# ZhengyiLuo/SMPLSim

Measured on AMD Instinct MI355X. Metric: env-steps/sec (whole node), 4096-env SMPL rollout at 1/2/4/8 MI355X, higher is better.
Workload: dtype f32

## Files before the change

include/smplsim_hip.h:

```cpp
#ifndef SMPLSIM_HIP_H
#define SMPLSIM_HIP_H
#include <stddef.h>
#include <stdint.h>

#ifdef __cplusplus
extern "C" {
#endif

typedef enum {
  SS_OK = 0,
  SS_ERR_INVALID = -1,
  SS_ERR_HIP = -2,
  SS_ERR_NOMEM = -3,
  SS_ERR_LDS = -4
} ss_status;

enum { SS_GEOM_BOX = 0, SS_GEOM_CAPSULE = 1,
       SS_GEOM_SPHERE = 2 };
enum { SS_TASK_BASE = 0, SS_TASK_SPEED = 1, SS_TASK_GETUP = 2, SS_TASK_REACH = 3 };
enum { SS_INIT_DEFAULT = 0, SS_INIT_FALL = 1,
       SS_INIT_EXTERNAL = 2 };
enum { SS_CTRL_UHC_PD = 0, SS_CTRL_PD = 1, SS_CTRL_TORQUE = 2, SS_CTRL_SIMPLE_PID = 3, SS_CTRL_DEFAULT = 4 };

typedef struct {
  int32_t nbody;
  const int32_t *body_parent;
  const double *body_pos;
  const double *body_mass;
  const double *body_ipos;
  const double *body_iquat;
  const double *body_inertia;
  const int32_t *geom_type;
  const double *geom_size;
  const double *geom_pos;
  const double *geom_quat;
  const double *dof_armature;
  const double *jnt_range;
  const uint8_t *jnt_limited;
  const double *body_invweight0;
  const double *dof_invweight0;
  const double *qpos0;
  int32_t nu;
  const int32_t *actuator_dof;
  const double *kp, *kd, *torque_lim, *act_scale, *act_offset;
  const uint8_t *legal_contact;
  double timestep, gravity, solref[2], solimp[5], margin, friction, impratio;
  const int32_t *geom_contype;
  const int32_t *geom_conaffinity;
  int32_t nexclude;
  const int32_t *exclude;
  double meaninertia;
} ss_model_desc;

typedef struct {
  int32_t task, state_init, self_obs_v, control_mode;
  int32_t episode_length, control_freq_inv, root_height_obs;
  float power_scale;
  float tar_speed_min, tar_speed_max; int32_t speed_change_min, speed_change_max;
  float tar_height_min, tar_height_max; int32_t height_change_min, height_change_max, recovery_steps;
  int32_t newton_iters;
  float tar_dist_max; int32_t reach_body;
  int32_t self_collision;
  float solver_tolerance;
} ss_env_cfg;
#ifndef SS_MAX_SELF_CONTACTS_N
#define SS_MAX_SELF_CONTACTS_N 64
#endif
enum { SS_MAX_SELF_CONTACTS = SS_MAX_SELF_CONTACTS_N };

typedef struct {
  int32_t num_envs;
  float *qpos;
  float *qvel;
  float *qpos_prev;
  float *qvel_prev;
  float *qacc_warm;
  float *body_vel;
  int32_t *touch;
  int32_t *cur_t;
  float *task;
  int32_t *nwarn;
  int32_t *solver_iters;
  float *pid_integral;
  float *pid_last_error;
  int32_t *pid_started;
  const int32_t *shape_id;
  int32_t *self_contacts;
} ss_state;

typedef struct ss_model ss_model;
typedef struct ss_batch ss_batch;

int ss_model_create(const ss_model_desc *desc, int device_id, ss_model **out);
int ss_model_create_shapes(const ss_model_desc *descs, int32_t num_shapes, int device_id, ss_model **out);

typedef struct {
  int32_t control_mode;
  int32_t clip_actions;
  double pdp_scale, pdd_scale;
  double timestep;
  int32_t num_contact_bodies;
  const char *const *contact_bodies;
} ss_mjcf_options;
int ss_model_create_from_mjcf(const char *xml, size_t len, const ss_mjcf_options *opts, int device_id, ss_model **out);
void ss_model_destroy(ss_model *m);
int ss_model_dims(const ss_model *m, int32_t *nq, int32_t *nv, int32_t *nu, int32_t *nbody);
int ss_model_elimination_tree(const ss_model *m, int32_t *root, int32_t *levels, int32_t *widest, int32_t *widths, int32_t *most_children);
int ss_obs_size(const ss_model *m, const ss_env_cfg *cfg);

int ss_batch_create(const ss_model *m, const ss_env_cfg *cfg, const ss_state *state, ss_batch **out);
void ss_batch_destroy(ss_batch *b);

int ss_reset(ss_batch *b, const uint8_t *mask, const float *fall_actions, const float *task_rand,
             float *obs, void *stream);

int ss_step(ss_batch *b, const float *actions, const float *task_rand, float *obs, float *reward,
            uint8_t *terminated, uint8_t *truncated, void *stream);

int ss_set_order(ss_batch *b, const int32_t *order);
int ss_schedule_longest_first(ss_batch *b, void *stream);

int ss_step_autoreset(ss_batch *b, const float *actions, const float *task_rand, const float *reset_task_rand, float *obs,
                      float *obs_next, float *reward, uint8_t *terminated, uint8_t *truncated, void *stream);
int ss_set_fall_actions(ss_batch *b, const float *fall_actions);

int ss_substep(ss_batch *b, const float *actions, int n_substeps, void *stream);

int ss_kinematics(ss_batch *b, float *xpos, float *xmat, void *stream);

int ss_set_body_outputs(ss_batch *b, float *xpos, float *xmat);

int ss_set_power_output(ss_batch *b, float *power);

int ss_debug_forward(ss_batch *b, const float *torques, float *M, float *bias, float *qacc, void *stream);
int ss_debug_self_contacts(ss_batch *b, float *records);
int ss_debug_self_truncation(ss_batch *b, int32_t *counts);
int ss_gae(const float *rewards, const float *not_done, const float *not_dead, const float *values, const float *bootstrap,
           int32_t T, int32_t N, float gamma, float tau, float *advantages, float *returns, void *stream);

int ss_debug_prof(ss_batch *b, unsigned long long *out, int n);

int ss_launch_info(const ss_batch *b, int32_t *envs_per_wg, int32_t *lds_bytes, int32_t *kernel_regs);

int ss_set_launch_geometry(ss_batch *b, int32_t envs_per_wg, int32_t max_workgroups);

enum { SS_FIELD_QPOS = 0,
       SS_FIELD_QVEL = 1,
       SS_FIELD_XPOS = 2,
       SS_FIELD_XMAT = 3,
       SS_FIELD_BODY_VEL = 4,
       SS_FIELD_TOUCH = 5,
       SS_FIELD_QACC_WARM = 6,
       SS_FIELD_CUR_T = 7 };
int ss_get_state(ss_batch *b, int32_t field, void *buf, void *stream);
int ss_set_state(ss_batch *b, int32_t field, const void *buf, void *stream);


const char *ss_last_error(void);
const char *ss_model_last_error(const ss_model *m);
const char *ss_batch_last_error(const ss_batch *b);

#ifdef __cplusplus
}
#endif
#endif
```

smplsim_amd/_cabi.py:

```python
import ctypes as C

import numpy as np

TASK_BASE, TASK_SPEED, TASK_GETUP, TASK_REACH = 0, 1, 2, 3
INIT_DEFAULT, INIT_FALL, INIT_EXTERNAL = 0, 1, 2
CTRL_UHC_PD, CTRL_PD, CTRL_TORQUE, CTRL_SIMPLE_PID, CTRL_DEFAULT = 0, 1, 2, 3, 4
TASKS = {"HumanoidEnv": TASK_BASE, "HumanoidSpeed": TASK_SPEED, "HumanoidGetup": TASK_GETUP, "HumanoidReach": TASK_REACH}
CONTROL_MODES = {"uhc_pd": CTRL_UHC_PD, "pd": CTRL_PD, "torque": CTRL_TORQUE, "simple_pid": CTRL_SIMPLE_PID,
                 "default": CTRL_DEFAULT}
STATE_INITS = {"Default": INIT_DEFAULT, "Fall": INIT_FALL, "External": INIT_EXTERNAL}
SS_MAX_SELF_CONTACTS = 64


class ModelDesc(C.Structure):
    _fields_ = [
        ("nbody", C.c_int32), ("body_parent", C.c_void_p), ("body_pos", C.c_void_p), ("body_mass", C.c_void_p),
        ("body_ipos", C.c_void_p), ("body_iquat", C.c_void_p), ("body_inertia", C.c_void_p),
        ("geom_type", C.c_void_p), ("geom_size", C.c_void_p), ("geom_pos", C.c_void_p), ("geom_quat", C.c_void_p),
        ("dof_armature", C.c_void_p), ("jnt_range", C.c_void_p), ("jnt_limited", C.c_void_p),
        ("body_invweight0", C.c_void_p), ("dof_invweight0", C.c_void_p), ("qpos0", C.c_void_p),
        ("nu", C.c_int32), ("actuator_dof", C.c_void_p), ("kp", C.c_void_p), ("kd", C.c_void_p),
        ("torque_lim", C.c_void_p), ("act_scale", C.c_void_p), ("act_offset", C.c_void_p),
        ("legal_contact", C.c_void_p),
        ("timestep", C.c_double), ("gravity", C.c_double), ("solref", C.c_double * 2), ("solimp", C.c_double * 5),
        ("margin", C.c_double), ("friction", C.c_double), ("impratio", C.c_double),
        ("geom_contype", C.c_void_p), ("geom_conaffinity", C.c_void_p), ("nexclude", C.c_int32), ("exclude", C.c_void_p),
        ("meaninertia", C.c_double),
    ]


class EnvCfg(C.Structure):
    _fields_ = [
        ("task", C.c_int32), ("state_init", C.c_int32), ("self_obs_v", C.c_int32), ("control_mode", C.c_int32),
        ("episode_length", C.c_int32), ("control_freq_inv", C.c_int32), ("root_height_obs", C.c_int32),
        ("power_scale", C.c_float),
        ("tar_speed_min", C.c_float), ("tar_speed_max", C.c_float), ("speed_change_min", C.c_int32),
        ("speed_change_max", C.c_int32),
        ("tar_height_min", C.c_float), ("tar_height_max", C.c_float), ("height_change_min", C.c_int32),
        ("height_change_max", C.c_int32), ("recovery_steps", C.c_int32), ("newton_iters", C.c_int32),
        ("tar_dist_max", C.c_float), ("reach_body", C.c_int32), ("self_collision", C.c_int32),
        ("solver_tolerance", C.c_float),
    ]


class State(C.Structure):
    _fields_ = [
        ("num_envs", C.c_int32), ("qpos", C.c_void_p), ("qvel", C.c_void_p), ("qpos_prev", C.c_void_p),
        ("qvel_prev", C.c_void_p), ("qacc_warm", C.c_void_p), ("body_vel", C.c_void_p), ("touch", C.c_void_p),
        ("cur_t", C.c_void_p), ("task", C.c_void_p), ("nwarn", C.c_void_p), ("solver_iters", C.c_void_p),
        ("pid_integral", C.c_void_p), ("pid_last_error", C.c_void_p), ("pid_started", C.c_void_p), ("shape_id", C.c_void_p),
        ("self_contacts", C.c_void_p),
    ]


class Skeleton(C.Structure):
    _fields_ = [("nbody", C.c_int32), ("parent", C.c_void_p), ("smpl_2_mujoco", C.c_void_p)]


MOTION_DATA_ARRAYS = ("length_starts", "motion_num_frames", "motion_dt", "motion_lengths", "frame_motion", "pose_aa", "trans",
                      "offsets", "gts", "grs", "lrs", "gvs", "gavs", "dof_pos", "dvs", "qpos", "qvel")


class MotionData(C.Structure):
    _fields_ = [("num_motions", C.c_int32), ("num_frames", C.c_int32), ("nbody", C.c_int32)] + \
               [(n, C.c_void_p) for n in MOTION_DATA_ARRAYS]


MOTION_STATE_FIELDS = ("root_pos", "root_rot", "dof_pos", "root_vel", "root_ang_vel", "dof_vel", "rg_pos", "rb_rot", "body_vel",
                       "body_ang_vel", "qpos", "qvel")


class MotionState(C.Structure):
    _fields_ = [(n, C.c_void_p) for n in MOTION_STATE_FIELDS]


class ImitationCfg(C.Structure):
    _fields_ = [(n, C.c_float) for n in ("k_pos", "k_rot", "k_vel", "k_ang_vel", "w_pos", "w_rot", "w_vel", "w_ang_vel",
                                         "termination_distance", "obs_dt")]


class ImitationIO(C.Structure):
    _fields_ = [("data", C.POINTER(MotionData)), ("cfg", ImitationCfg), ("motion_ids", C.c_void_p), ("start_times", C.c_void_p),
                ("offset", C.c_void_p), ("sampling_cdf", C.c_void_p), ("truncate_time", C.c_float), ("random_start", C.c_int32),
                ("obs_final", C.c_void_p), ("obs_next", C.c_void_p), ("obs_stride", C.c_int32), ("reward", C.c_void_p),
                ("reward_parts", C.c_void_p), ("terminated", C.c_void_p), ("truncated", C.c_void_p)]


class MjcfOptions(C.Structure):
    _fields_ = [("control_mode", C.c_int32), ("clip_actions", C.c_int32), ("pdp_scale", C.c_double), ("pdd_scale", C.c_double),
                ("timestep", C.c_double), ("num_contact_bodies", C.c_int32), ("contact_bodies", C.POINTER(C.c_char_p))]


def bind(lib):
    vp = C.c_void_p
    lib.ss_model_create_from_mjcf.argtypes = [C.c_char_p, C.c_size_t, C.POINTER(MjcfOptions), C.c_int, C.POINTER(vp)]
    lib.ss_set_fall_actions.argtypes = [vp, vp]
    lib.ss_get_state.argtypes = [vp, C.c_int32, vp, vp]
    lib.ss_set_state.argtypes = [vp, C.c_int32, vp, vp]
    lib.ss_imitation_bind.argtypes = [vp, C.POINTER(ImitationIO)]
    lib.ss_imitation_step_fused.argtypes = [vp, vp, vp, vp]
    lib.ss_model_last_error.argtypes = [vp]; lib.ss_model_last_error.restype = C.c_char_p
    lib.ss_batch_last_error.argtypes = [vp]; lib.ss_batch_last_error.restype = C.c_char_p
    lib.ss_model_create.argtypes = [C.POINTER(ModelDesc), C.c_int, C.POINTER(vp)]
    lib.ss_model_create_shapes.argtypes = [C.POINTER(ModelDesc), C.c_int32, C.c_int, C.POINTER(vp)]
    lib.ss_model_destroy.argtypes = [vp]; lib.ss_model_destroy.restype = None
    lib.ss_model_dims.argtypes = [vp] + [C.POINTER(C.c_int32)] * 4
    lib.ss_obs_size.argtypes = [vp, C.POINTER(EnvCfg)]
    lib.ss_batch_create.argtypes = [vp, C.POINTER(EnvCfg), C.POINTER(State), C.POINTER(vp)]
    lib.ss_batch_destroy.argtypes = [vp]; lib.ss_batch_destroy.restype = None
    lib.ss_reset.argtypes = [vp, vp, vp, vp, vp, vp]
    lib.ss_step.argtypes = [vp] * 8
    lib.ss_substep.argtypes = [vp, vp, C.c_int, vp]
    lib.ss_kinematics.argtypes = [vp, vp, vp, vp]
    lib.ss_debug_forward.argtypes = [vp, vp, vp, vp, vp, vp]
    lib.ss_debug_self_contacts.argtypes = [vp, vp]
    lib.ss_debug_self_truncation.argtypes = [vp, vp]
    lib.ss_model_elimination_tree.argtypes = [vp, vp, vp, vp, vp, vp]
    lib.ss_step_autoreset.argtypes = [vp] * 10
    lib.ss_schedule_longest_first.argtypes = [vp, vp]
    lib.ss_gae.argtypes = [vp, vp, vp, vp, vp, C.c_int32, C.c_int32, C.c_float, C.c_float, vp, vp, vp]
    lib.ss_debug_prof.argtypes = [vp, vp, C.c_int]
    lib.ss_set_order.argtypes = [vp, vp]
    lib.ss_set_body_outputs.argtypes = [vp, vp, vp]
    lib.ss_set_power_output.argtypes = [vp, vp]
    lib.ss_set_launch_geometry.argtypes = [vp, C.c_int32, C.c_int32]
    lib.ss_launch_info.argtypes = [vp] + [C.POINTER(C.c_int32)] * 3
    lib.ss_last_error.argtypes = []; lib.ss_last_error.restype = C.c_char_p
    lib.ss_motion_cook.argtypes = [C.POINTER(Skeleton), C.POINTER(MotionData), C.c_int32, vp]
    lib.ss_motion_state_at.argtypes = [C.POINTER(MotionData), vp, vp, vp, vp, C.c_int32, C.c_int32, C.POINTER(MotionState), vp]
    lib.ss_motion_resample.argtypes = [C.POINTER(MotionData), vp, vp, vp, C.c_float, C.c_int32, vp, vp, vp]
    lib.ss_imitation_step.argtypes = [C.POINTER(MotionData), C.POINTER(ImitationCfg)] + [vp] * 5 + [C.c_int32] + [vp] * 4 + \
                                     [C.c_int32] + [vp] * 5
    return lib


FIELDS = {"qpos": 0, "qvel": 1, "xpos": 2, "xmat": 3, "body_vel": 4, "touch": 5, "qacc_warm": 6, "cur_t": 7}
ACTIVATIONS = {"none": 0, "silu": 1, "tanh": 2, "relu": 3}
MLP_EXPORTS = ["ss_linear_bf16", "ss_linear_bf16_train", "ss_linear_bf16_dx", "ss_wgrad_bf16", "ss_obs_to_bf16", "ss_gaussian_sample",
               "ss_debug_last_gemm", "ss_linear_bf16_dx_det", "ss_linear_bf16_dx_det_workspace", "ss_wgrad_bf16_det", "ss_wgrad_bf16_det_workspace"]


def bind_mlp(lib):
    vp = C.c_void_p
    lib.ss_linear_bf16.argtypes = [vp, vp, vp, vp, C.c_int32, C.c_int32, C.c_int32, C.c_int32, C.c_int32, C.c_int32, vp]
    lib.ss_linear_bf16_train.argtypes = [vp, vp, vp, vp, vp, vp, vp, C.c_int32, C.c_int32, C.c_int32, C.c_int32, C.c_int32, C.c_int32, C.c_int32, vp]
    lib.ss_linear_bf16_dx.argtypes = [vp, vp, vp, vp, vp, C.c_int32, C.c_int32, C.c_int32, C.c_int32, vp]
    lib.ss_wgrad_bf16.argtypes = [vp, vp, vp, C.c_int32, C.c_int32, C.c_int32, C.c_int32, C.c_int32, C.c_int32, vp]
    lib.ss_linear_bf16_dx_det.argtypes = [vp, vp, vp, vp, vp, C.c_int32, C.c_int32, C.c_int32, C.c_int32, vp, C.c_int64, vp]
    lib.ss_linear_bf16_dx_det_workspace.argtypes = [C.c_int32, C.c_int32, C.c_int32]; lib.ss_linear_bf16_dx_det_workspace.restype = C.c_int64
    lib.ss_wgrad_bf16_det.argtypes = [vp, vp, vp, C.c_int32, C.c_int32, C.c_int32, C.c_int32, C.c_int32, C.c_int32, vp, C.c_int64, vp]
    lib.ss_wgrad_bf16_det_workspace.argtypes = [C.c_int32, C.c_int32, C.c_int32]; lib.ss_wgrad_bf16_det_workspace.restype = C.c_int64
    lib.ss_obs_to_bf16.argtypes = [vp, C.c_int32, C.c_int32, C.c_int32, vp, vp, vp, C.c_float, C.c_float, C.c_float, vp, C.c_int32, vp]
    lib.ss_gaussian_sample.argtypes = [vp, vp, vp, C.c_int32, C.c_int32, vp, C.c_int32, vp, C.c_int32, C.c_float, C.c_float, vp, vp]
    lib.ss_debug_last_gemm.argtypes = [C.c_char_p, C.c_int32]
    return lib


EXPORTS = ["ss_model_create", "ss_model_create_shapes", "ss_model_destroy", "ss_model_dims", "ss_model_elimination_tree", "ss_obs_size", "ss_batch_create",
           "ss_batch_destroy", "ss_reset", "ss_step", "ss_step_autoreset", "ss_substep", "ss_kinematics", "ss_debug_forward", "ss_debug_self_contacts", "ss_debug_self_truncation",
           "ss_gae", "ss_debug_prof", "ss_set_order", "ss_set_body_outputs", "ss_set_power_output", "ss_set_launch_geometry", "ss_schedule_longest_first", "ss_launch_info", "ss_last_error",
           "ss_model_create_from_mjcf", "ss_model_last_error", "ss_batch_last_error", "ss_imitation_bind", "ss_imitation_step_fused", "ss_get_state", "ss_set_state", "ss_set_fall_actions",
           "ss_motion_cook", "ss_motion_state_at", "ss_motion_resample", "ss_imitation_step"]


def make_model_desc(mc, kp, kd, torque_lim, act_scale, act_offset, legal_bodies=(), timestep=1.0 / 450):
    keep = []

    def arr(x, dt):
        a = np.ascontiguousarray(x, dtype=dt)
        keep.append(a)
        return a.ctypes.data_as(C.c_void_p)

    d = ModelDesc()
    d.nbody = mc.nbody
    d.body_parent = arr(mc.body_parent, np.int32)
    for name in ("body_pos", "body_mass", "body_ipos", "body_iquat", "body_inertia", "geom_size", "geom_pos",
                 "geom_quat", "dof_armature", "jnt_range", "body_invweight0", "dof_invweight0", "qpos0"):
        setattr(d, name, arr(getattr(mc, name), np.float64))
    d.geom_type = arr(mc.geom_type, np.int32)
    d.jnt_limited = arr(mc.jnt_limited, np.uint8)
    d.nu = mc.nu
    d.actuator_dof = arr(mc.actuator_dof, np.int32)
    d.kp, d.kd, d.torque_lim = arr(kp, np.float64), arr(kd, np.float64), arr(torque_lim, np.float64)
    d.act_scale, d.act_offset = arr(act_scale, np.float64), arr(act_offset, np.float64)
    d.legal_contact = arr([int(n in legal_bodies) for n in mc.body_names], np.uint8)
    d.timestep, d.gravity = timestep, mc.gravity
    d.solref = (C.c_double * 2)(*mc.solref)
    d.solimp = (C.c_double * 5)(*mc.solimp)
    d.margin, d.friction, d.impratio = mc.geom_margin, mc.friction, mc.impratio
    d.geom_contype = arr(mc.geom_contype, np.int32)
    d.geom_conaffinity = arr(mc.geom_conaffinity, np.int32)
    ex = [(mc.body_names.index(a), mc.body_names.index(b)) for a, b in mc.excludes]
    d.nexclude = len(ex)
    d.exclude = arr(np.array(ex, dtype=np.int32).reshape(-1, 2), np.int32) if ex else None
    d.meaninertia = mc.meaninertia
    return d, keep


def make_env_cfg(task=TASK_BASE, state_init=INIT_DEFAULT, self_obs_v=1, control_mode=CTRL_UHC_PD,
                 episode_length=300, control_freq_inv=15, root_height_obs=True, power_scale=1.0,
                 tar_speed=(0.0, 5.0), speed_change=(100, 200), tar_height=(0.5, 1.2), height_change=(100, 200),
                 recovery_steps=60, newton_iters=0, tar_dist_max=1.0, reach_body=0, self_collision=False, solver_tolerance=0.0):
    return EnvCfg(task, state_init, self_obs_v, control_mode, episode_length, control_freq_inv, int(root_height_obs),
                  power_scale, tar_speed[0], tar_speed[1], speed_change[0], speed_change[1], tar_height[0],
                  tar_height[1], height_change[0], height_change[1], recovery_steps, newton_iters, tar_dist_max, reach_body,
                  int(bool(self_collision)), solver_tolerance)
```

smplsim_amd/batch.py:

```python
import ctypes as C
import os
import warnings

import numpy as np
import torch

from . import _cabi
from ._lib import lib
from .gains import build_pd_tables
from .mjcf import compile_mjcf
from .mjcf_writer import default_xml_str

DEFAULT_CONTACT_BODIES = ("R_Ankle", "L_Ankle", "R_Toe", "L_Toe")


def _check(rc):
    if rc != 0:
        raise RuntimeError(f"libsmplsim_hip error {rc}: {lib().ss_last_error().decode()}")


def _ptr(t):
    return None if t is None else C.c_void_p(t.data_ptr())


def _shard_device(index):
    if not torch.cuda.is_available():
        raise RuntimeError("SMPLSimVecEnv needs a ROCm GPU (MI355X); there is no CPU fallback")
    return torch.device("cuda", int(index))


def _launch_stream(device):
    return C.c_void_p(torch.cuda.current_stream(device).cuda_stream)


_WARNED = False


def _warn_floor_only():
    global _WARNED
    if not _WARNED:
        _WARNED = True
        warnings.warn("SMPLSimVecEnv(self_collision=False): floor contacts and joint limits only — bodies of the humanoid pass through "
                      "each other, unlike mj_step on the reference MJCF (contype/conaffinity, smpl_humanoid.xml:5,24). Pass "
                      "self_collision=True for the reference's contact set (about 3x the step time under violent actions).", stacklevel=3)


class ShardModel:

    def __init__(self, xml=None, humanoid="smpl_humanoid", device=0, contact_bodies=DEFAULT_CONTACT_BODIES,
                 control_mode="uhc_pd", clip_actions=True, pdp_scale=1.0, pdd_scale=1.0, sim_timestep_inv=450, tables=None, xmls=None, mcs=None, compiler="python", lazy=False):
        if mcs is not None:
            self.mcs, self.xmls = list(mcs), []
            self.xml = None
        else:
            self.xmls = list(xmls) if xmls is not None else [xml if xml is not None else default_xml_str(humanoid)]
            self.xml = self.xmls[0]
            self.mcs = [compile_mjcf(x) for x in self.xmls]
        self.mc, self.num_shapes = self.mcs[0], len(self.mcs)
        rng = {n: self.mc.jnt_range[6 + i] for i, n in enumerate(self.mc.joint_names)}
        self.tables = tables if tables is not None else build_pd_tables(
            self.mc.actuator_names, lambda n: rng[n], clip_actions=clip_actions, control_mode=control_mode,
            pdp_scale=pdp_scale, pdd_scale=pdd_scale)
        self.device = int(device)
        if compiler == "native":
            if self.num_shapes != 1 or self.xml is None or tables is not None:
                raise ValueError("compiler='native' takes one MJCF text and the reference's gain table")
        elif compiler != "python":
            raise ValueError(f"unknown compiler {compiler!r}")
        self._args = dict(compiler=compiler, contact_bodies=tuple(contact_bodies), control_mode=control_mode, clip_actions=clip_actions,
                          pdp_scale=pdp_scale, pdd_scale=pdd_scale, sim_timestep_inv=sim_timestep_inv)
        self._handle, self._pid = None, None
        if not lazy:
            self.handle

    @property
    def handle(self):
        if self._handle is None or self._pid != os.getpid():
            a = self._args
            h = C.c_void_p()
            if a["compiler"] == "native":
                names = (C.c_char_p * len(a["contact_bodies"]))(*[n.encode() for n in a["contact_bodies"]])
                opt = _cabi.MjcfOptions(_cabi.CONTROL_MODES[a["control_mode"]], int(bool(a["clip_actions"])), a["pdp_scale"], a["pdd_scale"],
                                        1.0 / a["sim_timestep_inv"], len(a["contact_bodies"]), names)
                txt = self.xml.encode()
                _check(lib().ss_model_create_from_mjcf(txt, len(txt), C.byref(opt), self.device, C.byref(h)))
            else:
                descs, self._keep = (_cabi.ModelDesc * self.num_shapes)(), []
                for i, mc in enumerate(self.mcs):
                    descs[i], keep = _cabi.make_model_desc(mc, *self.tables, legal_bodies=a["contact_bodies"], timestep=1.0 / a["sim_timestep_inv"])
                    self._keep.append(keep)
                _check(lib().ss_model_create_shapes(descs, self.num_shapes, self.device, C.byref(h)))
            self._handle, self._pid = h, os.getpid()
        return self._handle

    def __del__(self):
        h = getattr(self, "_handle", None)
        if h and getattr(self, "_pid", None) == os.getpid():
            try:
                lib().ss_model_destroy(h)
            except Exception:
                pass


class SMPLSimVecEnv:

    def __init__(self, num_envs, model=None, device=0, task="HumanoidEnv", state_init="Default", self_obs_v=1,
                 control_mode="uhc_pd", episode_length=300, control_freq_inv=15, root_height_obs=True,
                 power_scale=1.0, tar_speed=(0.0, 5.0), speed_change=(100, 200), tar_height=(0.5, 1.2),
                 height_change=(100, 200), recovery_steps=60, tar_dist_max=1.0, reach_body="R_Hand", newton_iters=0, fused_autoreset=True,
                 autoreset=True, seed=0, lpt_order=True, shape_id=None, self_collision=False, solver_tolerance=0.0,
                 **model_kw):
        self.device = _shard_device(device if model is None else model.device)
        self.model = model if model is not None else ShardModel(device=device, control_mode=control_mode, **model_kw)
        mc = self.model.mc
        self.num_envs = int(num_envs)
        self.nq, self.nv, self.nu, self.nbody = mc.nq, mc.nv, mc.nu, mc.nbody
        self.task_id = _cabi.TASKS[task] if isinstance(task, str) else int(task)
        if self.task_id == _cabi.TASK_REACH and isinstance(reach_body, str) and reach_body not in mc.body_names:
            raise ValueError(f"reach_body {reach_body!r} is not a body of this model")
        self.state_init = _cabi.STATE_INITS[state_init] if isinstance(state_init, str) else int(state_init)
        if self.state_init == _cabi.INIT_EXTERNAL and autoreset:
            raise ValueError("StateInit External keeps the state the caller wrote: pass autoreset=False and reset finished envs "
                             "yourself (write qpos / qvel, then reset(mask)), as SMPLSimImitationVecEnv does")
        self.cfg = _cabi.make_env_cfg(
            task=self.task_id, state_init=self.state_init, self_obs_v=self_obs_v,
            control_mode=_cabi.CONTROL_MODES[control_mode], episode_length=episode_length,
            control_freq_inv=control_freq_inv, root_height_obs=root_height_obs, power_scale=power_scale,
            tar_speed=tar_speed, speed_change=speed_change, tar_height=tar_height, height_change=height_change,
            recovery_steps=recovery_steps, newton_iters=newton_iters, tar_dist_max=tar_dist_max,
            reach_body=self._body_index(mc, reach_body), self_collision=self_collision, solver_tolerance=solver_tolerance)
        self.self_collision = bool(self_collision)
        if not self.self_collision:
            _warn_floor_only()
        N, dev = self.num_envs, self.device
        f32 = dict(dtype=torch.float32, device=dev)
        i32 = dict(dtype=torch.int32, device=dev)
        self.qpos = torch.zeros(N, self.nq, **f32); self.qvel = torch.zeros(N, self.nv, **f32)
        self.qpos_prev = torch.zeros(N, self.nq, **f32); self.qvel_prev = torch.zeros(N, self.nv, **f32)
        self.qacc_warm = torch.zeros(N, self.nv, **f32); self.body_vel = torch.zeros(N, self.nbody, 6, **f32)
        self.touch = torch.zeros(N, 2, **i32); self.cur_t = torch.zeros(N, **i32)
        self.task_state = torch.zeros(N, 4, **f32); self.nwarn = torch.zeros(N, **i32)
        self.solver_iters = torch.zeros(N, **i32)
        self.pid_integral = torch.zeros(N, self.nu, **f32); self.pid_last_error = torch.zeros(N, self.nu, **f32)
        self.pid_started = torch.zeros(N, **i32)
        self.self_contacts = torch.zeros(N, **i32)
        self.qpos[:, 3] = 1; self.qpos_prev[:, 3] = 1
        self.shape_id = None
        if self.model.num_shapes > 1:
            sid = torch.arange(N, device=dev) % self.model.num_shapes if shape_id is None else torch.as_tensor(shape_id, device=dev)
            if sid.shape != (N,) or int(sid.min()) < 0 or int(sid.max()) >= self.model.num_shapes:
                raise ValueError("shape_id must hold one shape index in [0, num_shapes) per env")
            self.shape_id = sid.to(torch.int32).contiguous()
        elif shape_id is not None:
            raise ValueError("shape_id given but the model has a single shape (build it with ShardModel(xmls=[...]))")
        st = _cabi.State(N, *[_ptr(t) for t in (self.qpos, self.qvel, self.qpos_prev, self.qvel_prev, self.qacc_warm,
                                               self.body_vel, self.touch, self.cur_t, self.task_state, self.nwarn,
                                               self.solver_iters, self.pid_integral, self.pid_last_error,
                                               self.pid_started, self.shape_id, self.self_contacts)])
        self.handle = C.c_void_p()
        _check(lib().ss_batch_create(self.model.handle, C.byref(self.cfg), C.byref(st), C.byref(self.handle)))
        self.obs_size = lib().ss_obs_size(self.model.handle, C.byref(self.cfg))
        self.obs_buf = torch.zeros(N, self.obs_size, **f32)
        self.rew_buf = torch.zeros(N, **f32)
        self.terminated = torch.zeros(N, dtype=torch.uint8, device=dev)
        self.truncated = torch.zeros(N, dtype=torch.uint8, device=dev)
        self.reset_buf = torch.zeros(N, dtype=torch.uint8, device=dev)
        self.obs_final = torch.zeros(N, self.obs_size, **f32)
        self._fused_autoreset = self.state_init in (_cabi.INIT_DEFAULT, _cabi.INIT_FALL) and fused_autoreset
        self._fall_buf = None
        if self._fused_autoreset and self.state_init == _cabi.INIT_FALL:
            self._fall_buf = torch.zeros(N, 3, self.nu, **f32)
            _check(lib().ss_set_fall_actions(self.handle, _ptr(self._fall_buf)))
        self.autoreset = autoreset
        self.gen = torch.Generator(device=dev)
        self.gen.manual_seed(int(seed))
        self.action_size = self.nu
        self.actuator_names = list(mc.actuator_names)
        self._keep = self._keep2 = None
        self.lpt_order = bool(lpt_order) and N > 64
        self.order = torch.arange(N, dtype=torch.int32, device=dev)

    @staticmethod
    def _body_index(mc, body):
        if not isinstance(body, str):
            return int(body)
        if body in mc.body_names:
            return mc.body_names.index(body)
        return 0

    def _task_rand(self):
        if self.task_id == _cabi.TASK_BASE:
            return None
        return torch.rand(self.num_envs, 4, generator=self.gen, device=self.device)

    def _fall_actions(self):
        if self.state_init != _cabi.INIT_FALL:
            return None
        return torch.rand(self.num_envs, 3, self.nu, generator=self.gen, device=self.device)

    def _stream(self):
        return _launch_stream(self.device)

    def reset(self, mask=None, fall_actions=None, task_rand=None):
        fa = fall_actions if fall_actions is not None else self._fall_actions()
        tr = task_rand if task_rand is not None else self._task_rand()
        m = None if mask is None else mask.to(torch.uint8).contiguous()
        self._keep = (fa, tr, m)
        _check(lib().ss_reset(self.handle, _ptr(m), _ptr(fa), _ptr(tr), _ptr(self.obs_buf), self._stream()))
        return self.obs_buf, {"critic_state": self.obs_buf}

    def step(self, actions, task_rand=None, _events=None, task_rand2=None, _fall_drawn=False):
        actions = actions.to(torch.float32).contiguous()
        assert actions.shape == (self.num_envs, self.nu) and actions.device == self.device
        tr = task_rand if task_rand is not None else self._task_rand()
        self._keep = (actions, tr)
        if self.lpt_order:
            _check(lib().ss_schedule_longest_first(self.handle, self._stream()))
        if _events:
            _events[0].record()
        info = {}
        if self.autoreset and self._fused_autoreset:
            tr2 = task_rand2 if task_rand2 is not None else self._task_rand()
            self._keep2 = (tr2,)
            if self._fall_buf is not None and not _fall_drawn:
                self._fall_buf.uniform_(0.0, 1.0, generator=self.gen)
            _check(lib().ss_step_autoreset(self.handle, _ptr(actions), _ptr(tr), _ptr(tr2), _ptr(self.obs_final), _ptr(self.obs_buf),
                                           _ptr(self.rew_buf), _ptr(self.terminated), _ptr(self.truncated), self._stream()))
            if _events:
                _events[1].record()
            if self.lpt_order:
                _check(lib().ss_set_order(self.handle, None))
            info["final_observation"] = self.obs_final
            info["critic_state"] = self.obs_buf
            return self.obs_buf, self.rew_buf, self.terminated.bool(), self.truncated.bool(), info
        _check(lib().ss_step(self.handle, _ptr(actions), _ptr(tr), _ptr(self.obs_buf), _ptr(self.rew_buf),
                             _ptr(self.terminated), _ptr(self.truncated), self._stream()))
        if _events:
            _events[1].record()
        if self.lpt_order:
            _check(lib().ss_set_order(self.handle, None))
        if self.autoreset:
            torch.bitwise_or(self.terminated, self.truncated, out=self.reset_buf)
            info["final_observation"] = self.obs_buf.clone()
            fa, tr2 = self._fall_actions(), self._task_rand()
            self._keep2 = (fa, tr2)
            _check(lib().ss_reset(self.handle, _ptr(self.reset_buf), _ptr(fa), _ptr(tr2), _ptr(self.obs_buf),
                                  self._stream()))
        info["critic_state"] = self.obs_buf
        return self.obs_buf, self.rew_buf, self.terminated.bool(), self.truncated.bool(), info

    def substep(self, actions, n):
        actions = actions.to(torch.float32).contiguous()
        self._keep = (actions,)
        _check(lib().ss_substep(self.handle, _ptr(actions), int(n), self._stream()))

    def kinematics(self):
        xpos = torch.zeros(self.num_envs, self.nbody, 3, device=self.device)
        xmat = torch.zeros(self.num_envs, self.nbody, 9, device=self.device)
        _check(lib().ss_kinematics(self.handle, _ptr(xpos), _ptr(xmat), self._stream()))
        return xpos, xmat

    def enable_power_usage(self):
        if getattr(self, "power_usage", None) is None:
            self.power_usage = torch.zeros(self.num_envs, int(self.cfg.control_freq_inv), self.nv - 6, device=self.device)
            _check(lib().ss_set_power_output(self.handle, _ptr(self.power_usage)))
        return self.power_usage

    def debug_forward(self, torques=None):
        M = torch.zeros(self.num_envs, self.nv, self.nv, device=self.device)
        bias = torch.zeros(self.num_envs, self.nv, device=self.device)
        qacc = torch.zeros(self.num_envs, self.nv, device=self.device)
        tq = None if torques is None else torques.to(torch.float32).contiguous()
        _check(lib().ss_debug_forward(self.handle, _ptr(tq), _ptr(M), _ptr(bias), _ptr(qacc), self._stream()))
        return M, bias, qacc

    def debug_self_contacts(self):
        if getattr(self, "self_records", None) is None:
            self.self_records = torch.zeros(self.num_envs, _cabi.SS_MAX_SELF_CONTACTS, 24, device=self.device)
            _check(lib().ss_debug_self_contacts(self.handle, _ptr(self.self_records)))
        return self.self_records

    def set_state(self, qpos, qvel, qpos_prev=None, qvel_prev=None, warm=None):
        def as_t(x):
            if torch.is_tensor(x):
                return x.to(self.device, torch.float32)
            return torch.as_tensor(np.asarray(x), dtype=torch.float32, device=self.device)
        self.qpos.copy_(as_t(qpos)); self.qvel.copy_(as_t(qvel))
        self.qpos_prev.copy_(as_t(qpos if qpos_prev is None else qpos_prev))
        self.qvel_prev.copy_(as_t(qvel if qvel_prev is None else qvel_prev))
        if warm is not None:
            self.qacc_warm.copy_(as_t(warm))

    def launch_info(self):
        a, b, c = C.c_int32(), C.c_int32(), C.c_int32()
        _check(lib().ss_launch_info(self.handle, C.byref(a), C.byref(b), C.byref(c)))
        return {"envs_per_workgroup": a.value, "lds_bytes": b.value, "vgprs": c.value}

    def close(self):
        h = getattr(self, "handle", None)
        if h:
            if self.device.type == "cuda":
                torch.cuda.synchronize(self.device)
            lib().ss_batch_destroy(h)
            self.handle = None

    def __del__(self):
        try:
            self.close()
        except Exception:
            pass
```

smplsim_amd/csrc/smplsim_hip.hip:

```cpp
#include <hip/hip_runtime.h>

#include "ss_env_kernel.h"

namespace {


__global__ void ss_gae_kernel(const float *rew, const float *nd, const float *ndead, const float *val, const float *boot,
                              int T, int N, float gamma, float tau, float *adv, float *ret) {
  const int n = blockIdx.x * blockDim.x + threadIdx.x;
  if (n >= N) return;
  float next_v = boot ? boot[n] : 0.f, next_a = 0.f;
  for (int t = T - 1; t >= 0; --t) {
    const size_t i = (size_t)t * N + n;
    const float v = val[i];
    const float delta = rew[i] + gamma * next_v * ndead[i] - v;
    const float a = delta + gamma * tau * next_a * nd[i];
    adv[i] = a; ret[i] = v + a;
    next_v = v; next_a = a;
  }
}

__global__ void __launch_bounds__(256) ss_key_kernel(const float *qvel, const float *qacc, const int32_t *touch, const int32_t *iters, int nv, int n,
                                                     int32_t *key) {
  const int env = blockIdx.x * 4 + (threadIdx.x >> 6), lane = threadIdx.x & 63;
  if (env >= n) return;
  float vm = 0.f, am = 0.f;
  for (int i = lane; i < nv; i += 64) {
    const float v = fabsf(qvel[(size_t)env * nv + i]), a = fabsf(qacc[(size_t)env * nv + i]);
    vm = fmaxf(vm, v == v ? v : 1e6f); am = fmaxf(am, a == a ? a : 1e12f);
  }
  for (int m = 32; m >= 1; m >>= 1) { vm = fmaxf(vm, __shfl_xor(vm, m, 64)); am = fmaxf(am, __shfl_xor(am, m, 64)); }
  if (lane == 0) {
    const int tc = __popc((unsigned)touch[2 * env]) + __popc((unsigned)touch[2 * env + 1]);
    const float k = (float)iters[env] + 6.f * (float)tc + 8.f * log1pf(fminf(am, 1e12f)) + 8.f * log1pf(fminf(vm, 1e6f));
    key[env] = (int32_t)fminf(fmaxf(k, 0.f), 1023.f);
  }
}

__global__ void __launch_bounds__(1024) ss_order_kernel(const int32_t *keys, int32_t *order, int n) {
  __shared__ int hist[1024], offs[1024];
  for (int i = threadIdx.x; i < 1024; i += blockDim.x) hist[i] = 0;
  __syncthreads();
  for (int i = threadIdx.x; i < n; i += blockDim.x) { int key = keys[i]; key = key < 0 ? 0 : (key > 1023 ? 1023 : key); atomicAdd(&hist[1023 - key], 1); }
  __syncthreads();
  if (threadIdx.x < 32) {
    int acc = 0;
    for (int i = 0; i < 32; i++) { const int h_ = hist[threadIdx.x * 32 + i]; offs[threadIdx.x * 32 + i] = acc; acc += h_; }
    int base = 0;
    for (int l = 0; l < 32; l++) { const int t = __shfl(acc, l, 64); if (l < (int)threadIdx.x) base += t; }
    for (int i = 0; i < 32; i++) offs[threadIdx.x * 32 + i] += base;
  }
  __syncthreads();
  for (int i = threadIdx.x; i < n; i += blockDim.x) { int key = keys[i]; key = key < 0 ? 0 : (key > 1023 ? 1023 : key); order[atomicAdd(&offs[1023 - key], 1)] = i; }
}


typedef ss::kern_t kern_t;
kern_t pick_kernel(int variant, int flavour, const ss::Hdr &h, const ss::HdrC &hc) {
#ifndef SS_NO_FIXED_LAYOUT
  if (variant == 0 && flavour == 0 && HdrSmpl::matches(h, hc)) return ss_env_kernel<2, 2, 1, 1, SS_MAX_THREADS, false, false, HdrSmpl>;
#ifndef SS_ONLY_HEADLINE
  if (variant == 0 && flavour == 1 && HdrSmpl::matches(h, hc)) return ss_env_kernel<2, 2, 1, 1, SS_MAX_THREADS, true, false, HdrSmpl>;
  if (variant == 0 && flavour == 2 && HdrSmpl::matches(h, hc)) return ss_env_kernel<2, 2, 1, 1, SS_MAX_THREADS, true, true, HdrSmpl>;
#endif
#endif
  if (variant == 0 && flavour == 0) return ss_env_kernel<2, 2, 1, 1, SS_MAX_THREADS, false, false>;
#ifndef SS_ONLY_HEADLINE
  if (flavour == 3 || flavour == 5 || flavour == 7) return ss::pick_kernel_selfcol(variant, flavour == 5, flavour == 7, h, hc);
  if (flavour == 4 || flavour == 6) return ss::pick_kernel_imitation(variant, flavour == 6, h, hc);
  if (variant == 0) {
    if (flavour == 1) return ss_env_kernel<2, 2, 1, 1, SS_MAX_THREADS, true, false>;
    return ss_env_kernel<2, 2, 1, 1, SS_MAX_THREADS, true, true>;
  }
  if (variant == 1) return ss::pick_kernel_x(flavour, h, hc);
#endif
  return nullptr;
}

struct HipBackend {
  static void *alloc(size_t n) { void *p = nullptr; return hipMalloc(&p, n) == hipSuccess ? p : nullptr; }
  static void free_(void *p) { if (p) (void)hipFree(p); }
  static bool upload(void *dst, const void *src, size_t n) { return hipMemcpy(dst, src, n, hipMemcpyHostToDevice) == hipSuccess; }
  static bool set_device(int d) { return hipSetDevice(d) == hipSuccess; }
  static bool download(void *dst, const void *src, size_t n) { return hipMemcpy(dst, src, n, hipMemcpyDeviceToHost) == hipSuccess; }
  static bool copy_d2d(void *dst, const void *src, size_t n, void *stream) { return hipMemcpyAsync(dst, src, n, hipMemcpyDeviceToDevice, (hipStream_t)stream) == hipSuccess; }
  static int lds_capacity() { return 160 * 1024; }
  static int num_cus() { int d = 0, n = 256; if (hipGetDevice(&d) == hipSuccess) { hipDeviceProp_t p; if (hipGetDeviceProperties(&p, d) == hipSuccess) n = p.multiProcessorCount; } return n; }
  static int max_waves(int variant, int selfcol) { return (variant == 0 ? (selfcol ? SS_MAX_THREADS_SC : SS_MAX_THREADS) : SS_MAX_THREADS_X) / 64; }
  static const char *order_by_key(const ss_state &st, int nv, int32_t *key, int32_t *order, void *stream) {
    const int n = st.num_envs;
    hipLaunchKernelGGL(ss_key_kernel, dim3((n + 3) / 4), dim3(256), 0, (hipStream_t)stream, st.qvel, st.qacc_warm, st.touch, st.solver_iters, nv, n, key);
    hipLaunchKernelGGL(ss_order_kernel, dim3(1), dim3(1024), 0, (hipStream_t)stream, key, order, n);
    hipError_t e = hipGetLastError();
    return e == hipSuccess ? nullptr : hipGetErrorString(e);
  }
  static const char *gae(const float *rew, const float *nd, const float *ndead, const float *val, const float *boot, int T, int N,
                         float gamma, float tau, float *adv, float *ret, void *stream) {
    hipLaunchKernelGGL(ss_gae_kernel, dim3((N + 255) / 256), dim3(256), 0, (hipStream_t)stream, rew, nd, ndead, val, boot, T, N, gamma, tau, adv, ret);
    hipError_t e = hipGetLastError();
    return e == hipSuccess ? nullptr : hipGetErrorString(e);
  }
  static int &regs_ref() { static thread_local int r = 0; return r; }
  static int kernel_regs() { return regs_ref(); }
  static const char *launch(const ss::KArgs &k, int nenv, int envs_per_wg, size_t lds_bytes, void *stream, int fixed_epw, int max_wgs) {
    const bool bodyout = (k.out0 || k.power) && (k.mode == ss::MODE_STEP || k.mode == ss::MODE_RESET);
    const int flavour = k.im ? (k.cfg.self_collision ? 7 : (k.st.shape_id ? 6 : 4)) : (k.cfg.self_collision ? (k.st.shape_id ? 5 : 3) : (k.st.shape_id ? 2 : (bodyout ? 1 : 0)));
    kern_t kern = pick_kernel(ss::kernel_variant(k.h), flavour, k.h, k.hc);
    if (!kern) return "no kernel variant for this model size";
    static thread_local kern_t configured[32] = {};
    static thread_local size_t configured_lds[32] = {};
    static thread_local int regs_by_slot[32] = {};
    const int slot = 16 * ss::kernel_variant(k.h) + flavour;
    if (configured[slot] != kern || configured_lds[slot] < lds_bytes) {
      hipError_t e = hipFuncSetAttribute(reinterpret_cast<const void *>(kern), hipFuncAttributeMaxDynamicSharedMemorySize, (int)lds_bytes);
      if (e != hipSuccess) return hipGetErrorString(e);
      hipFuncAttributes fa;
      if (hipFuncGetAttributes(&fa, reinterpret_cast<const void *>(kern)) == hipSuccess) regs_by_slot[slot] = fa.numRegs;
      configured[slot] = kern; configured_lds[slot] = lds_bytes;
    }
    regs_ref() = regs_by_slot[slot];
    static thread_local int cus = num_cus();
    const int per_cu = (nenv + cus - 1) / cus;
    if (fixed_epw > 0) {
      envs_per_wg = fixed_epw;
      lds_bytes = ss::launch_lds_bytes(k, envs_per_wg);
    } else if (per_cu < envs_per_wg) {
      envs_per_wg = per_cu < 1 ? 1 : per_cu;
      lds_bytes = ss::launch_lds_bytes(k, envs_per_wg);
    }
    int wgs = (nenv + envs_per_wg - 1) / envs_per_wg;
    const int resident = cus * (int)(lds_capacity() / lds_bytes > 0 ? lds_capacity() / lds_bytes : 1);
    if (wgs > resident) wgs = resident;
    if (max_wgs > 0 && wgs > max_wgs) wgs = max_wgs;
    dim3 grid(wgs), block(64 * envs_per_wg);
    hipLaunchKernelGGL(kern, grid, block, lds_bytes, (hipStream_t)stream, k);
    hipError_t e = hipGetLastError();
    return e == hipSuccess ? nullptr : hipGetErrorString(e);
  }
};

}

SS_DEFINE_C_API(HipBackend)
```

smplsim_amd/csrc/ss_api.h:

```cpp
#pragma once
#include <cstdlib>
#include <new>
#include <string>

#include "ss_imfused.h"
#include "ss_mjcf.h"
#include "ss_tables.h"

namespace ss {
inline std::string &last_error() { static thread_local std::string e; return e; }
inline std::string *&error_slot() { static thread_local std::string *p = nullptr; return p; }
struct HandleScope {
  explicit HandleScope(std::string *slot) { error_slot() = slot; }
  ~HandleScope() { error_slot() = nullptr; }
};
}

struct ss_model {
  ss::HostModel hm;
  int device = 0;
  uint32_t *d_shared = nullptr;
  ss::real *d_bodyc = nullptr, *d_candc = nullptr;
  int32_t *d_candb = nullptr;
  int32_t *d_pairs = nullptr;
  ss::real *d_geomc = nullptr;
  int num_shapes = 1;
  mutable std::string err;
};
struct ss_batch {
  const ss_model *m = nullptr;
  ss_env_cfg cfg{};
  ss_state st{};
  int envs_per_wg = 1;
  size_t lds_bytes = 0;
  int obs_size = 0;
  int32_t *d_counter = nullptr;
  unsigned long long *d_prof = nullptr;
  const int32_t *order = nullptr;
  int32_t *d_sched = nullptr;
  float *body_xpos = nullptr, *body_xmat = nullptr;
  static ss::real *R(float *p) { return reinterpret_cast<ss::real *>(p); }
  static const ss::real *R(const float *p) { return reinterpret_cast<const ss::real *>(p); }
  float *dbg_self = nullptr;
  int32_t *self_trunc = nullptr;
  float *power = nullptr;
  int fixed_envs_per_wg = 0, max_wgs = 0;
  mutable std::string err;
  mutable int kernel_regs = 0;
  mutable int parity = 0;
  float *d_kin = nullptr;
  const float *fall_actions = nullptr;
  void *d_im = nullptr;
  ss_imitation_io im_io{};
};

inline bool same_pair_ids(const std::vector<int32_t> &a, const std::vector<int32_t> &b) {
  if (a.size() != b.size()) return false;
  for (size_t i = 0; i < a.size(); i += 2) if (a[i] != b[i]) return false;
  return true;
}

template <class BE>
struct ss_api {
  static int fail(int code, const std::string &msg) {
    ss::last_error() = msg;
    if (ss::error_slot()) *ss::error_slot() = msg;
    return code;
  }

  static int model_create(const ss_model_desc *d, int device, ss_model **out) {
    if (!d || !out) return fail(SS_ERR_INVALID, "null argument");
    ss_model *m = new (std::nothrow) ss_model();
    if (!m) return fail(SS_ERR_NOMEM, "out of host memory");
    if (!ss::build_host_model(*d, m->hm)) { std::string e = m->hm.error; delete m; return fail(SS_ERR_INVALID, e); }
    m->device = device;
    if (!BE::set_device(device)) { delete m; return fail(SS_ERR_HIP, "cannot select device"); }
    auto up = [&](const void *src, size_t bytes) -> void * {
      void *p = BE::alloc(bytes ? bytes : 4);
      if (p && bytes && !BE::upload(p, src, bytes)) { BE::free_(p); p = nullptr; }
      return p;
    };
    m->d_shared = (uint32_t *)up(m->hm.shared.data(), m->hm.shared.size() * 4);
    m->d_bodyc = (ss::real *)up(m->hm.bodyc.data(), m->hm.bodyc.size() * sizeof(ss::real));
    m->d_candc = (ss::real *)up(m->hm.candc.data(), m->hm.candc.size() * sizeof(ss::real));
    m->d_candb = (int32_t *)up(m->hm.candb.data(), m->hm.candb.size() * 4);
    {
      std::vector<int32_t> pt(m->hm.pairs);
      m->hm.sc.o_sctab = (int)pt.size();
      pt.insert(pt.end(), m->hm.sctab.begin(), m->hm.sctab.end());
      m->d_pairs = (int32_t *)up(pt.data(), pt.size() * 4);
    }
    m->d_geomc = (ss::real *)up(m->hm.geomc.data(), m->hm.geomc.size() * sizeof(ss::real));
    if (!m->d_shared || !m->d_bodyc || !m->d_candc || !m->d_candb || !m->d_pairs || !m->d_geomc) { model_destroy(m); return fail(SS_ERR_HIP, "device table upload failed"); }
    *out = m;
    return SS_OK;
  }
  static int model_create_shapes(const ss_model_desc *d, int num_shapes, int device, ss_model **out) {
    if (!d || !out || num_shapes < 1) return fail(SS_ERR_INVALID, "null argument or num_shapes < 1");
    if (num_shapes == 1) return model_create(d, device, out);
    ss_model *m = new (std::nothrow) ss_model();
    if (!m) return fail(SS_ERR_NOMEM, "out of host memory");
    std::vector<ss::real> bodyc, candc, geomc;
    std::vector<int32_t> pairs;
    for (int s = 0; s < num_shapes; s++) {
      ss::HostModel hm;
      if (!ss::build_host_model(d[s], hm)) { std::string e = "shape " + std::to_string(s) + ": " + hm.error; delete m; return fail(SS_ERR_INVALID, e); }
      const ss::Hdr &h = hm.h;
      std::vector<ss::real> iw(h.nv);
      ss::real *sf = ss::shared_reals(hm);
      for (int i = 0; i < h.nv; i++) { iw[i] = sf[h.o_dofc + i * ss::kDofC + 4]; sf[h.o_dofc + i * ss::kDofC + 4] = 0; }
      for (int i = 0; i < 3 * h.nb; i++) sf[h.o_boff + i] = 0;
      if (s == 0) m->hm = hm;
      else {
        const ss::Hdr &g = m->hm.h;
        const bool same = h.nb == g.nb && h.nv == g.nv && h.nu == g.nu && h.ncand == g.ncand && h.nbox == g.nbox && h.nslot == g.nslot &&
                          h.shared_words == g.shared_words && h.env_floats == g.env_floats && hm.shared == m->hm.shared &&
                          hm.candb == m->hm.candb && same_pair_ids(hm.pairs, m->hm.pairs) && hm.illegal_mask == m->hm.illegal_mask && h.dt == g.dt && h.grav == g.grav &&
                          h.margin == g.margin && h.mu == g.mu && h.K == g.K && h.B == g.B;
        if (!same) { delete m; return fail(SS_ERR_INVALID, "shape " + std::to_string(s) + " differs from shape 0 in more than its geometry"); }
      }
      bodyc.insert(bodyc.end(), hm.bodyc.begin(), hm.bodyc.end());
      iw.resize((h.nv + 3) & ~3, ss::real(0));
      bodyc.insert(bodyc.end(), iw.begin(), iw.end());
      candc.insert(candc.end(), hm.candc.begin(), hm.candc.end());
      geomc.insert(geomc.end(), hm.geomc.begin(), hm.geomc.end());
      pairs.insert(pairs.end(), hm.pairs.begin(), hm.pairs.end());
    }
    if (12 * m->hm.h_sc.nb > m->hm.h_sc.l_Wst - m->hm.h_sc.l_IA) { delete m; return fail(SS_ERR_LDS, "no room for the per-env body offsets"); }
    m->device = device; m->num_shapes = num_shapes;
    if (!BE::set_device(device)) { delete m; return fail(SS_ERR_HIP, "cannot select device"); }
    auto up = [&](const void *src, size_t bytes) -> void * {
      void *p = BE::alloc(bytes ? bytes : 4);
      if (p && bytes && !BE::upload(p, src, bytes)) { BE::free_(p); p = nullptr; }
      return p;
    };
    m->d_shared = (uint32_t *)up(m->hm.shared.data(), m->hm.shared.size() * 4);
    m->d_bodyc = (ss::real *)up(bodyc.data(), bodyc.size() * sizeof(ss::real));
    m->d_candc = (ss::real *)up(candc.data(), candc.size() * sizeof(ss::real));
    m->d_candb = (int32_t *)up(m->hm.candb.data(), m->hm.candb.size() * 4);
    m->hm.sc.o_sctab = (int)pairs.size();
    pairs.insert(pairs.end(), m->hm.sctab.begin(), m->hm.sctab.end());
    m->d_pairs = (int32_t *)up(pairs.data(), pairs.size() * 4);
    m->d_geomc = (ss::real *)up(geomc.data(), geomc.size() * sizeof(ss::real));
    if (!m->d_shared || !m->d_bodyc || !m->d_candc || !m->d_candb || !m->d_pairs || !m->d_geomc) { model_destroy(m); return fail(SS_ERR_HIP, "device table upload failed"); }
    *out = m;
    return SS_OK;
  }
  static void model_destroy(ss_model *m) {
    if (!m) return;
    BE::free_(m->d_shared); BE::free_(m->d_bodyc); BE::free_(m->d_candc); BE::free_(m->d_candb); BE::free_(m->d_pairs); BE::free_(m->d_geomc);
    delete m;
  }
  static int batch_create(const ss_model *m, const ss_env_cfg *cfg, const ss_state *st, ss_batch **out) {
    if (!m || !cfg || !st || !out) return fail(SS_ERR_INVALID, "null argument");
    if (st->num_envs < 1) return fail(SS_ERR_INVALID, "num_envs must be positive");
    if (!st->qpos || !st->qvel || !st->qpos_prev || !st->qvel_prev || !st->qacc_warm || !st->body_vel || !st->touch ||
        !st->cur_t || !st->task || !st->nwarn || !st->solver_iters)
      return fail(SS_ERR_INVALID, "every ss_state buffer must be provided");
    if (cfg->control_mode < SS_CTRL_UHC_PD || cfg->control_mode > SS_CTRL_DEFAULT) return fail(SS_ERR_INVALID, "unknown control_mode");
    if (cfg->control_mode == SS_CTRL_SIMPLE_PID && (!st->pid_integral || !st->pid_last_error || !st->pid_started))
      return fail(SS_ERR_INVALID, "control_mode simple_pid needs the pid_* state buffers");
    if (cfg->self_obs_v != 1 && cfg->self_obs_v != 2) return fail(SS_ERR_INVALID, "self_obs_v must be 1 or 2");
    if (cfg->control_freq_inv < 1) return fail(SS_ERR_INVALID, "control_freq_inv must be >= 1");
    if (m->num_shapes > 1 && !st->shape_id) return fail(SS_ERR_INVALID, "a model with several shapes needs ss_state.shape_id");
    if (m->num_shapes == 1 && st->shape_id) return fail(SS_ERR_INVALID, "ss_state.shape_id given for a single-shape model");
    if (cfg->self_collision && !m->d_pairs) return fail(SS_ERR_INVALID, "model has no pair table");
    if (cfg->self_collision && !m->hm.self_collision_unavailable.empty()) return fail(SS_ERR_INVALID, m->hm.self_collision_unavailable.c_str());
    if (cfg->task == SS_TASK_REACH && (cfg->reach_body < 0 || cfg->reach_body >= m->hm.h.nb)) return fail(SS_ERR_INVALID, "reach_body out of range");
    const ss::Hdr &h = m->hm.h;
    if (ss::kernel_variant(h) < 0) return fail(SS_ERR_INVALID, "model too large for the compiled kernel variants");
    ss_batch *b = new (std::nothrow) ss_batch();
    if (!b) return fail(SS_ERR_NOMEM, "out of host memory");
    b->m = m; b->cfg = *cfg; b->st = *st;
    if (b->cfg.newton_iters <= 0) b->cfg.newton_iters = 100;
    b->cfg.solver_tolerance = (float)((cfg->solver_tolerance > 0.f ? (double)cfg->solver_tolerance : 1e-8) * m->hm.meaninertia * (h.nv > 1 ? h.nv : 1));
    b->obs_size = ss::obs_size(h, *cfg);
    size_t shared_b = (size_t)((h.shared_words + 3) & ~3) * 4;
    const size_t env_b = (size_t)(cfg->self_collision ? m->hm.sc.env_floats : h.env_floats) * sizeof(ss::real);
    int cap = BE::lds_capacity();
    const size_t pool_b = cfg->self_collision ? (size_t)ss::ss_pool_floats(m->hm.sc) * sizeof(ss::real) : 0;
    int e = (int)((cap - (long)shared_b - (long)pool_b) / (long)env_b);
    if (e < 1) { delete b; return fail(SS_ERR_LDS, "model does not fit in LDS"); }
    { const int mw = BE::max_waves(ss::kernel_variant(h), cfg->self_collision); if (e > mw) e = mw; }
    { const char *cap = getenv("SS_ENVS_PER_WG"); if (cap && atoi(cap) > 0 && atoi(cap) < e) e = atoi(cap); }
    b->envs_per_wg = e;
    b->lds_bytes = shared_b + (size_t)e * env_b + pool_b;
#ifdef SS_PROFILE
    b->d_prof = (unsigned long long *)BE::alloc(64 * sizeof(unsigned long long));
    if (b->d_prof) { unsigned long long z[64] = {0}; BE::upload(b->d_prof, z, sizeof z); }
#endif
    if (!BE::set_device(m->device)) { delete b; return fail(SS_ERR_HIP, "cannot select device"); }
    b->d_counter = (int32_t *)BE::alloc(2 * sizeof(int32_t));
    const int32_t zeros[2] = {0, 0};
    if (!b->d_counter || !BE::upload(b->d_counter, zeros, sizeof zeros)) { BE::free_(b->d_counter); delete b; return fail(SS_ERR_NOMEM, "device allocation failed"); }
    *out = b;
    return SS_OK;
  }
  static ss::KArgs base_args(const ss_batch *b, int mode) {
    ss::KArgs k{};
    const ss_model *m = b->m;
    k.h = b->cfg.self_collision ? m->hm.h_sc : m->hm.h; k.cfg = b->cfg; k.st = b->st;
    k.shared_g = m->d_shared; k.bodyc = m->d_bodyc; k.candc = m->d_candc; k.candb = m->d_candb;
    k.illegal_mask = m->hm.illegal_mask;
    k.hc = m->hm.hc;
    k.sc = m->hm.sc; k.pairs = m->d_pairs; k.geomc = m->d_geomc; k.dbg_self = ss_batch::R(b->dbg_self);
    k.mode = mode; k.nsub = b->cfg.control_freq_inv; k.obs_size = b->obs_size;
    k.work_counter = b->d_counter + b->parity; k.work_counter_next = b->d_counter + (b->parity ^ 1);
    k.obs_stride = b->obs_size;
    k.prof = b->d_prof;
    k.order = b->order;
    if (mode == ss::MODE_STEP || mode == ss::MODE_RESET) { k.out0 = ss_batch::R(b->body_xpos); k.out1 = ss_batch::R(b->body_xmat); }
    if (mode == ss::MODE_STEP) { k.power = ss_batch::R(b->power); k.self_trunc = b->self_trunc; }
    return k;
  }
  static int run(const ss_batch *b, const ss::KArgs &k, void *stream) {
    if (!BE::set_device(b->m->device)) return fail(SS_ERR_HIP, "cannot select device");
    const char *err = BE::launch(k, b->st.num_envs, b->envs_per_wg, b->lds_bytes, stream, b->fixed_envs_per_wg, b->max_wgs);
    if (err) return fail(SS_ERR_HIP, err);
    b->kernel_regs = BE::kernel_regs();
    b->parity ^= 1;
    return SS_OK;
  }
  static int reset(ss_batch *b, const uint8_t *mask, const float *fall_actions, const float *task_rand, float *obs, void *stream) {
    if (!b || !obs) return fail(SS_ERR_INVALID, "null argument");
    if (b->cfg.state_init == SS_INIT_FALL && !fall_actions) return fail(SS_ERR_INVALID, "StateInit.Fall needs fall_actions");
    ss::KArgs k = base_args(b, ss::MODE_RESET);
    k.mask = mask; k.fall_actions = ss_batch::R(fall_actions); k.task_rand = ss_batch::R(task_rand); k.obs = ss_batch::R(obs);
    return run(b, k, stream);
  }
  static int step(ss_batch *b, const float *actions, const float *task_rand, float *obs, float *reward, uint8_t *term,
                  uint8_t *trunc, void *stream) {
    if (!b || !actions || !obs || !reward || !term || !trunc) return fail(SS_ERR_INVALID, "null argument");
    ss::KArgs k = base_args(b, ss::MODE_STEP);
    k.actions = ss_batch::R(actions); k.task_rand = ss_batch::R(task_rand); k.obs = ss_batch::R(obs); k.reward = ss_batch::R(reward);
    k.terminated = term; k.truncated = trunc;
    return run(b, k, stream);
  }
  static int step_autoreset(ss_batch *b, const float *actions, const float *task_rand, const float *reset_task_rand, float *obs,
                            float *obs_next, float *reward, uint8_t *term, uint8_t *trunc, void *stream) {
    if (!b || !actions || !obs || !obs_next || !reward || !term || !trunc) return fail(SS_ERR_INVALID, "null argument");
    if (b->cfg.state_init == SS_INIT_EXTERNAL) return fail(SS_ERR_INVALID, "in-launch autoreset: StateInit External has no reset state of its own");
    if (b->cfg.state_init == SS_INIT_FALL && !b->fall_actions) return fail(SS_ERR_INVALID, "in-launch Fall reset needs ss_set_fall_actions");
    ss::KArgs k = base_args(b, ss::MODE_STEP);
    k.actions = ss_batch::R(actions); k.task_rand = ss_batch::R(task_rand); k.obs = ss_batch::R(obs); k.reward = ss_batch::R(reward);
    k.terminated = term; k.truncated = trunc;
    k.fused_reset = 1; k.obs2 = ss_batch::R(obs_next); k.task_rand2 = ss_batch::R(reset_task_rand);
    if (b->cfg.state_init == SS_INIT_FALL) k.fall_actions = ss_batch::R(b->fall_actions);
    return run(b, k, stream);
  }
  static int imitation_bind(ss_batch *b, const ss_imitation_io *io) {
    if (!b || !io) return fail(SS_ERR_INVALID, "null argument");
    if (sizeof(ss::real) != sizeof(float)) return fail(SS_ERR_INVALID, "not available in the float64 build");
    if (const char *e = ss::mo::check_data(io->data, false)) return fail(SS_ERR_INVALID, e);
    const ss::Hdr &h = b->m->hm.h;
    if (io->data->nbody != h.nb) return fail(SS_ERR_INVALID, "motion data and model disagree on nbody");
    if (b->cfg.state_init != SS_INIT_EXTERNAL || b->cfg.task != SS_TASK_BASE)
      return fail(SS_ERR_INVALID, "the fused imitation step needs a batch with task base and StateInit External");
    if (b->cfg.self_collision && (b->st.shape_id || ss::kernel_variant(h) != 0))
      return fail(SS_ERR_INVALID, "fused imitation step with self_collision: SMPL-sized single-shape models only (use the separate launches)");
    if (!b->body_xpos || !b->body_xmat) return fail(SS_ERR_INVALID, "call ss_set_body_outputs first");
    if (!io->motion_ids || !io->start_times || !io->obs_final || !io->obs_next || !io->reward || !io->terminated || !io->truncated)
      return fail(SS_ERR_INVALID, "null buffer in ss_imitation_io");
    if (io->obs_stride < b->obs_size + 24 * h.nb) return fail(SS_ERR_INVALID, "obs_stride smaller than self + task observation");
    if (io->truncate_time < 0.f) return fail(SS_ERR_INVALID, "truncate_time must be >= 0");
    ss::mo::ImFused f{};
    f.im = ss::mo::ImArgs{*io->data, io->cfg, io->motion_ids, io->start_times, b->st.cur_t, io->offset, nullptr, b->st.num_envs,
                          b->body_xpos, b->body_xmat, b->st.body_vel, io->obs_final + b->obs_size, io->obs_stride, io->reward,
                          io->reward_parts, io->terminated, io->truncated};
    f.ids = io->motion_ids; f.start_times = io->start_times; f.cdf = io->sampling_cdf; f.truncate = io->truncate_time;
    f.random_start = io->random_start; f.obs_final = io->obs_final; f.obs_next = io->obs_next;
    f.obs_floats = b->obs_size + 24 * h.nb; f.qpos = b->st.qpos; f.qvel = b->st.qvel; f.nq = h.nq; f.nv = h.nv;
    if (!BE::set_device(b->m->device)) return fail(SS_ERR_HIP, "cannot select device");
    if (!b->d_im) b->d_im = BE::alloc(sizeof f);
    if (!b->d_im || !BE::upload(b->d_im, &f, sizeof f)) return fail(SS_ERR_NOMEM, "device allocation failed");
    b->im_io = *io;
    return SS_OK;
  }
  static int imitation_step_fused(ss_batch *b, const float *actions, const float *rand, void *stream) {
    if (!b || !actions) return fail(SS_ERR_INVALID, "null argument");
    if (!b->d_im) return fail(SS_ERR_INVALID, "ss_imitation_bind first");
    if (rand && !b->im_io.sampling_cdf) return fail(SS_ERR_INVALID, "re-initialisation needs ss_imitation_io.sampling_cdf");
    ss::KArgs k = base_args(b, ss::MODE_STEP);
    k.actions = ss_batch::R(actions);
    k.obs = ss_batch::R(b->im_io.obs_final); k.obs2 = ss_batch::R(b->im_io.obs_next); k.obs_stride = b->im_io.obs_stride;
    k.im = b->d_im; k.im_rand = rand;
    return run(b, k, stream);
  }
  static int state_field(ss_batch *b, int field, void *buf, bool set, void *stream) {
    if (!b || !buf) return fail(SS_ERR_INVALID, "null argument");
    if (sizeof(ss::real) != sizeof(float)) return fail(SS_ERR_INVALID, "not available in the float64 build");
    const ss::Hdr &h = b->m->hm.h;
    const size_t N = (size_t)b->st.num_envs;
    if (!BE::set_device(b->m->device)) return fail(SS_ERR_HIP, "cannot select device");
    auto copy = [&](void *mine, size_t bytes) { return (set ? BE::copy_d2d(mine, buf, bytes, stream) : BE::copy_d2d(buf, mine, bytes, stream)) ? SS_OK : fail(SS_ERR_HIP, "device copy failed"); };
    switch (field) {
      case SS_FIELD_QPOS: {
        if (int rc = copy(b->st.qpos, N * h.nq * 4)) return rc;
        return set ? (BE::copy_d2d(b->st.qpos_prev, buf, N * h.nq * 4, stream) ? SS_OK : fail(SS_ERR_HIP, "device copy failed")) : SS_OK;
      }
      case SS_FIELD_QVEL: {
        if (int rc = copy(b->st.qvel, N * h.nv * 4)) return rc;
        return set ? (BE::copy_d2d(b->st.qvel_prev, buf, N * h.nv * 4, stream) ? SS_OK : fail(SS_ERR_HIP, "device copy failed")) : SS_OK;
      }
      case SS_FIELD_QACC_WARM: return copy(b->st.qacc_warm, N * h.nv * 4);
      case SS_FIELD_CUR_T: return copy(b->st.cur_t, N * 4);
      default: break;
    }
    if (set) return fail(SS_ERR_INVALID, "ss_set_state: field is read-only (QPOS, QVEL, QACC_WARM, CUR_T can be set)");
    switch (field) {
      case SS_FIELD_BODY_VEL: return copy(b->st.body_vel, N * h.nb * 6 * 4);
      case SS_FIELD_TOUCH: return copy(b->st.touch, N * 2 * 4);
      case SS_FIELD_XPOS: case SS_FIELD_XMAT: {
        if (!b->d_kin) b->d_kin = (float *)BE::alloc(N * h.nb * 12 * 4);
        if (!b->d_kin) return fail(SS_ERR_NOMEM, "device allocation failed");
        float *xp = b->d_kin, *xm = b->d_kin + N * h.nb * 3;
        if (int rc = kinematics(b, xp, xm, stream)) return rc;
        return field == SS_FIELD_XPOS ? copy(xp, N * h.nb * 3 * 4) : copy(xm, N * h.nb * 9 * 4);
      }
      default: return fail(SS_ERR_INVALID, "unknown state field");
    }
  }
  static int substep(ss_batch *b, const float *actions, int n, void *stream) {
    if (!b || !actions || n < 1) return fail(SS_ERR_INVALID, "bad argument");
    ss::KArgs k = base_args(b, ss::MODE_SUBSTEP);
    k.actions = ss_batch::R(actions); k.nsub = n;
    return run(b, k, stream);
  }
  static int kinematics(ss_batch *b, float *xpos, float *xmat, void *stream) {
    if (!b || !xpos || !xmat) return fail(SS_ERR_INVALID, "null argument");
    ss::KArgs k = base_args(b, ss::MODE_KINEMATICS);
    k.out0 = ss_batch::R(xpos); k.out1 = ss_batch::R(xmat);
    return run(b, k, stream);
  }
  static int debug_forward(ss_batch *b, const float *torques, float *M, float *bias, float *qacc, void *stream) {
    if (!b || !M || !bias || !qacc) return fail(SS_ERR_INVALID, "null argument");
    ss::KArgs k = base_args(b, ss::MODE_DEBUG_FORWARD);
    k.actions = ss_batch::R(torques); k.out0 = ss_batch::R(M); k.out1 = ss_batch::R(bias); k.out2 = ss_batch::R(qacc);
    return run(b, k, stream);
  }
};

#define SS_DEFINE_C_API(BE)                                                                                          \
  extern "C" {                                                                                                       \
  int ss_model_create(const ss_model_desc *d, int dev, ss_model **out) { return ss_api<BE>::model_create(d, dev, out); } \
  int ss_model_create_shapes(const ss_model_desc *d, int32_t n, int dev, ss_model **out) { return ss_api<BE>::model_create_shapes(d, n, dev, out); } \
  void ss_model_destroy(ss_model *m) { ss_api<BE>::model_destroy(m); }                                               \
  int ss_model_dims(const ss_model *m, int32_t *nq, int32_t *nv, int32_t *nu, int32_t *nb) {                          \
    ss::HandleScope hs_(m ? &m->err : nullptr);                                                                      \
    if (!m) return ss_api<BE>::fail(SS_ERR_INVALID, "null model");                                                   \
    if (nq) *nq = m->hm.h.nq;                                                                                        \
    if (nv) *nv = m->hm.h.nv;                                                                                        \
    if (nu) *nu = m->hm.h.nu;                                                                                        \
    if (nb) *nb = m->hm.h.nb;                                                                                        \
    return SS_OK;                                                                                                    \
  }                                                                                                                  \
  int ss_model_elimination_tree(const ss_model *m, int32_t *root, int32_t *levels, int32_t *widest, int32_t *widths, int32_t *most_children) { \
    ss::HandleScope hs_(m ? &m->err : nullptr);                                                                      \
    if (!m) return ss_api<BE>::fail(SS_ERR_INVALID, "null model");                                                   \
    const ss::HdrC &c = m->hm.hc;                                                                                    \
    if (root) *root = c.root;                                                                                        \
    if (levels) *levels = c.nlev;                                                                                    \
    if (widest) *widest = m->hm.h.maxlev;                                                                            \
    if (widths) {                                                                                                    \
      widths[0] = c.pel_level;                                                                                       \
      for (int L = 1; L <= c.nlev && L <= 32; L++) widths[L] = (int)((c.nkpack[(L - 1) >> 4] >> (4 * ((L - 1) & 15))) & 15ull) + 1; \
    }                                                                                                                \
    if (most_children) most_children[0] = (int)((c.chain & 0xffffull) | ((c.neg & 0x7fffull) << 16));                                            \
    if (most_children) for (int L = 1; L <= c.nlev && L <= 32; L++) most_children[L] = (L <= 21 && c.cpack != ~0ull) ? (int)((c.cpack >> (3 * (L - 1))) & 7ull) : -1; \
    return SS_OK;                                                                                                    \
  }                                                                                                                  \
  int ss_obs_size(const ss_model *m, const ss_env_cfg *c) { return (m && c) ? ss::obs_size(m->hm.h, *c) : SS_ERR_INVALID; } \
  int ss_batch_create(const ss_model *m, const ss_env_cfg *c, const ss_state *s, ss_batch **o) { ss::HandleScope hs_(m ? &m->err : nullptr); return ss_api<BE>::batch_create(m, c, s, o); } \
  void ss_batch_destroy(ss_batch *b) { if (b) { BE::free_(b->d_kin); BE::free_(b->d_im); BE::free_(b->d_counter); BE::free_(b->d_prof); BE::free_(b->d_sched); delete b; } }          \
  int ss_set_order(ss_batch *b, const int32_t *order) { ss::HandleScope hs_(b ? &b->err : nullptr);                                                              \
    if (!b) return ss_api<BE>::fail(SS_ERR_INVALID, "null batch");                                                  \
    b->order = order; return SS_OK;                                                                                  \
  }                                                                                                                  \
  int ss_set_launch_geometry(ss_batch *b, int32_t envs_per_wg, int32_t max_workgroups) { ss::HandleScope hs_(b ? &b->err : nullptr);                              \
    if (!b || envs_per_wg < 0 || envs_per_wg > b->envs_per_wg || max_workgroups < 0)                                   \
      return ss_api<BE>::fail(SS_ERR_INVALID, "envs per workgroup must be in [0, ss_launch_info's value], max_workgroups >= 0"); \
    b->fixed_envs_per_wg = envs_per_wg; b->max_wgs = max_workgroups; return SS_OK;                                     \
  }                                                                                                                  \
  int ss_set_body_outputs(ss_batch *b, float *xpos, float *xmat) { ss::HandleScope hs_(b ? &b->err : nullptr);                                                    \
    if (!b || (!xpos) != (!xmat)) return ss_api<BE>::fail(SS_ERR_INVALID, "pass both buffers or neither");           \
    b->body_xpos = xpos; b->body_xmat = xmat; return SS_OK;                                                          \
  }                                                                                                                  \
  int ss_set_power_output(ss_batch *b, float *power) { ss::HandleScope hs_(b ? &b->err : nullptr);                                                               \
    if (!b) return ss_api<BE>::fail(SS_ERR_INVALID, "null batch");                                                  \
    b->power = power; return SS_OK;                                                                                  \
  }                                                                                                                  \
  int ss_debug_self_truncation(ss_batch *b, int32_t *counts) { ss::HandleScope hs_(b ? &b->err : nullptr);                                                       \
    if (!b) return ss_api<BE>::fail(SS_ERR_INVALID, "null batch");                                                  \
    b->self_trunc = counts; return SS_OK;                                                                            \
  }                                                                                                                  \
  int ss_debug_self_contacts(ss_batch *b, float *records) { ss::HandleScope hs_(b ? &b->err : nullptr);                                                           \
    if (!b) return ss_api<BE>::fail(SS_ERR_INVALID, "null batch");                                                  \
    b->dbg_self = records; return SS_OK;                                                                             \
  }                                                                                                                  \
  int ss_schedule_longest_first(ss_batch *b, void *stream) { ss::HandleScope hs_(b ? &b->err : nullptr);                                                        \
    if (!b) return ss_api<BE>::fail(SS_ERR_INVALID, "null batch");                                                  \
    if (!BE::set_device(b->m->device)) return ss_api<BE>::fail(SS_ERR_HIP, "cannot select device");                  \
    if (!b->d_sched) b->d_sched = (int32_t *)BE::alloc(2 * sizeof(int32_t) * (size_t)b->st.num_envs);                  \
    if (!b->d_sched) return ss_api<BE>::fail(SS_ERR_NOMEM, "device allocation failed");                              \
    const char *err = BE::order_by_key(b->st, b->m->hm.h.nv, b->d_sched + b->st.num_envs, b->d_sched, stream);         \
    if (err) return ss_api<BE>::fail(SS_ERR_HIP, err);                                                               \
    b->order = b->d_sched; return SS_OK;                                                                             \
  }                                                                                                                  \
  int ss_gae(const float *rew, const float *nd, const float *ndead, const float *val, const float *boot, int32_t T,   \
             int32_t N, float gamma, float tau, float *adv, float *ret, void *stream) {                             \
    if (!rew || !nd || !ndead || !val || !adv || !ret) return ss_api<BE>::fail(SS_ERR_INVALID, "null argument");     \
    if (T < 1 || N < 1) return ss_api<BE>::fail(SS_ERR_INVALID, "T and N must be positive");                         \
    const char *err = BE::gae(rew, nd, ndead, val, boot, T, N, gamma, tau, adv, ret, stream);                         \
    return err ? ss_api<BE>::fail(SS_ERR_HIP, err) : SS_OK;                                                          \
  }                                                                                                                  \
  int ss_debug_prof(ss_batch *b, unsigned long long *out, int n) { ss::HandleScope hs_(b ? &b->err : nullptr);                                                   \
    if (!b || !out || !b->d_prof) return ss_api<BE>::fail(SS_ERR_INVALID, "not a profiling build");                 \
    return BE::download(out, b->d_prof, (size_t)n * 8) ? SS_OK : SS_ERR_HIP;                                         \
  }                                                                   \
  int ss_reset(ss_batch *b, const uint8_t *mask, const float *fa, const float *tr, float *obs, void *st) { ss::HandleScope hs_(b ? &b->err : nullptr); return ss_api<BE>::reset(b, mask, fa, tr, obs, st); } \
  int ss_step(ss_batch *b, const float *a, const float *tr, float *obs, float *rew, uint8_t *te, uint8_t *tu, void *st) { ss::HandleScope hs_(b ? &b->err : nullptr); return ss_api<BE>::step(b, a, tr, obs, rew, te, tu, st); } \
  int ss_step_autoreset(ss_batch *b, const float *a, const float *tr, const float *tr2, float *obs, float *obs_next, float *rew, \
                        uint8_t *te, uint8_t *tu, void *st) { ss::HandleScope hs_(b ? &b->err : nullptr); return ss_api<BE>::step_autoreset(b, a, tr, tr2, obs, obs_next, rew, te, tu, st); } \
  int ss_set_fall_actions(ss_batch *b, const float *fa) {                                                             \
    if (!b) return ss_api<BE>::fail(SS_ERR_INVALID, "null batch");                                                  \
    b->fall_actions = fa; return SS_OK;                                                                              \
  }                                                                                                                  \
  int ss_get_state(ss_batch *b, int32_t field, void *buf, void *st) { ss::HandleScope hs_(b ? &b->err : nullptr); return ss_api<BE>::state_field(b, field, buf, false, st); } \
  int ss_set_state(ss_batch *b, int32_t field, const void *buf, void *st) { ss::HandleScope hs_(b ? &b->err : nullptr); return ss_api<BE>::state_field(b, field, const_cast<void *>(buf), true, st); } \
  int ss_imitation_bind(ss_batch *b, const ss_imitation_io *io) { ss::HandleScope hs_(b ? &b->err : nullptr); return ss_api<BE>::imitation_bind(b, io); } \
  int ss_imitation_step_fused(ss_batch *b, const float *a, const float *rand, void *st) { ss::HandleScope hs_(b ? &b->err : nullptr); return ss_api<BE>::imitation_step_fused(b, a, rand, st); } \
  int ss_substep(ss_batch *b, const float *a, int n, void *st) { ss::HandleScope hs_(b ? &b->err : nullptr); return ss_api<BE>::substep(b, a, n, st); }          \
  int ss_kinematics(ss_batch *b, float *xpos, float *xmat, void *st) { ss::HandleScope hs_(b ? &b->err : nullptr); return ss_api<BE>::kinematics(b, xpos, xmat, st); } \
  int ss_debug_forward(ss_batch *b, const float *tq, float *M, float *bias, float *qacc, void *st) { ss::HandleScope hs_(b ? &b->err : nullptr); return ss_api<BE>::debug_forward(b, tq, M, bias, qacc, st); } \
  int ss_launch_info(const ss_batch *b, int32_t *epw, int32_t *lds, int32_t *regs) { ss::HandleScope hs_(b ? &b->err : nullptr);                                 \
    if (!b) return ss_api<BE>::fail(SS_ERR_INVALID, "null batch");                                                   \
    if (epw) *epw = b->envs_per_wg;                                                                                  \
    if (lds) *lds = (int32_t)b->lds_bytes;                                                                           \
    if (regs) *regs = b->kernel_regs;                                                                                \
    return SS_OK;                                                                                                    \
  }                                                                                                                  \
  const char *ss_last_error(void) { return ss::last_error().c_str(); }                                               \
  const char *ss_model_last_error(const ss_model *m) { return m ? m->err.c_str() : ""; }                               \
  const char *ss_batch_last_error(const ss_batch *b) { return b ? b->err.c_str() : ""; }                               \
  int ss_model_create_from_mjcf(const char *xml, size_t len, const ss_mjcf_options *opt, int dev, ss_model **out) {   \
    if (!xml || !out) return ss_api<BE>::fail(SS_ERR_INVALID, "null argument");                                      \
    ss::mjcf::Compiled c; std::string e;                                                                             \
    if (!ss::mjcf::compile(xml, len ? len : std::strlen(xml), opt, c, e)) return ss_api<BE>::fail(SS_ERR_INVALID, "MJCF: " + e); \
    return ss_api<BE>::model_create(&c.desc, dev, out);                                                              \
  }                                                                                                                  \
  }
```

smplsim_amd/csrc/ss_env_kernel.h:

```cpp
#pragma once
#include <hip/hip_runtime.h>

#include "ss_api.h"
#include "ss_kernel.h"
#include "ss_wave_gpu.h"

#ifndef SS_MAX_THREADS
#define SS_MAX_THREADS 768
#endif
#ifndef SS_MAX_THREADS_X
#define SS_MAX_THREADS_X 448
#endif
#ifndef SS_MAX_THREADS_SC
#define SS_MAX_THREADS_SC 512
#endif

namespace ss {
typedef void (*kern_t)(const KArgs);
kern_t pick_kernel_selfcol(int variant, bool shaped, bool imit, const Hdr &h, const HdrC &hc);
kern_t pick_kernel_imitation(int variant, bool shaped, const Hdr &h, const HdrC &hc);
kern_t pick_kernel_imitation_selfcol(int variant, bool shaped, const Hdr &h, const HdrC &hc);
kern_t pick_kernel_x(int flavour, const Hdr &h, const HdrC &hc);
}

namespace {

template <int DOFP, int CANDP, int SLOTP, int NPASS, int MAXT, bool BODYOUT, bool SHAPED, class HT = ss::HdrRuntime, bool SELFCOL = false, bool IMIT = false>
__global__ void __launch_bounds__(MAXT) ss_env_kernel(const ss::KArgs k) {
  extern __shared__ __align__(16) uint32_t lds[];
  if (blockIdx.x == 0 && threadIdx.x == 0) *k.work_counter_next = 0;
  for (int i = threadIdx.x; i < k.h.shared_words; i += blockDim.x) lds[i] = k.shared_g[i];
  if constexpr (SELFCOL)
    if (threadIdx.x == 0 && ss::ss_pool_floats(k.sc) > 0)
      *reinterpret_cast<int *>(reinterpret_cast<float *>(lds + ((k.h.shared_words + 3) & ~3)) + (size_t)(blockDim.x >> 6) * k.sc.env_floats) = 0;
  __syncthreads();
  const int wave = __builtin_amdgcn_readfirstlane(threadIdx.x >> 6);
  const int slice = SELFCOL ? k.sc.env_floats : HT::view(k.h).env_floats;
  float *L = reinterpret_cast<float *>(lds + ((k.h.shared_words + 3) & ~3)) + (size_t)wave * slice;
  float *pool = nullptr;
  if constexpr (SELFCOL) {
    if (ss::ss_pool_floats(k.sc) > 0) {
      pool = reinterpret_cast<float *>(lds + ((k.h.shared_words + 3) & ~3)) + (size_t)(blockDim.x >> 6) * slice;
    }
  }
  WaveGpu w{(int)(threadIdx.x & 63)};
  const int total_waves = (int)(gridDim.x * (blockDim.x >> 6));
  bool first = true;
  for (;;) {
    int env = wave * (int)gridDim.x + (int)blockIdx.x;
    if (!first) {
      if (w.ln == 0) env = atomicAdd(k.work_counter, 1) + total_waves;
      env = __builtin_amdgcn_readfirstlane(env);
    }
    first = false;
    if (env >= k.st.num_envs) break;
    if (k.order) env = __builtin_amdgcn_readfirstlane(k.order[env]);
    int mode = k.mode;
    if constexpr (IMIT) {
      const ss::mo::ImFused *f = static_cast<const ss::mo::ImFused *>(k.im);
      ss::run_env<WaveGpu, DOFP, CANDP, SLOTP, NPASS, BODYOUT, SHAPED, HT, SELFCOL>(&w, &k, lds, L, env, mode, pool);
      w.sync();
      if (ss::mo::fused_after_step(&w, f, k.im_rand, env)) {
        ss::run_env<WaveGpu, DOFP, CANDP, SLOTP, NPASS, BODYOUT, SHAPED, HT, SELFCOL>(&w, &k, lds, L, env, ss::MODE_RESET, pool);
        w.sync();
        ss::mo::fused_after_reset(&w, f, env);
      }
      continue;
    }
    for (int rep = 0; rep < 2; rep++) {
      const bool again = ss::run_env<WaveGpu, DOFP, CANDP, SLOTP, NPASS, BODYOUT, SHAPED, HT, SELFCOL>(&w, &k, lds, L, env, mode, pool);
      w.sync();
      if (!again) break;
      mode = ss::MODE_RESET;
    }
  }
}


typedef ss::HdrSmplFixed HdrSmpl;
typedef ss::HdrSmplxFixed HdrSmplx;

}
```

smplsim_amd/csrc/ss_hdr.h:

```cpp
#pragma once
#include <stdint.h>

#include "../../include/smplsim_hip.h"

#ifdef SS_F64
namespace ss { typedef double real; }
#define SS_M(fn) fn
#define SS_LS_TOL_EFF 1e-13
#define SS_ROUND_REL 2.2e-15
#define SS_DG_NOISE 1.8e-15
#define SS_LS_MAXIT 60
#else
namespace ss { typedef float real; }
#define SS_M(fn) fn##f
#define SS_LS_TOL_EFF SS_LS_TOL
#define SS_ROUND_REL 2e-6f
#define SS_DG_NOISE 1e-6f
#define SS_LS_MAXIT 16
#endif

namespace ss {

constexpr int kWave = 64;
constexpr int kBodyC = 16;
constexpr int kDofC = 12;
constexpr int kCandC = 8;

struct Hdr {
  int nb, nn, nv, nq, nu, ncand, nlev, a_stride, nbox, nslot, maxlev;
  int l_Rloc, l_w2;
  unsigned long long arm_lean;
  int o_dofc, o_boff, o_chainnode, o_ndepth, l_act, o_bparent, o_sumsmall, o_sumbig, o_sumcover, n_sumsmall, n_sumbig, shared_words;
  int l_q, l_v, l_a, l_tau, l_Fb, l_Pb, l_delta, l_diag, l_S, l_Ab, l_An, l_Aown, l_IA, l_Ubuf, l_Wst,
      l_R, l_r, l_Gb, l_tmp, l_V, l_Iown, ia_stride, env_floats;
  real dt, grav, margin, mu, solimp[5], K, B;
  real qpos0_root[3];
};

struct Layout {
  int l_q, l_v, l_a, l_tau, l_Fb, l_Pb, l_delta, l_diag, l_S, l_Ab, l_An, l_Aown, l_IA, l_Ubuf, l_Wst, l_R, l_r, l_Gb, l_tmp, l_V, l_Iown,
      ia_stride, l_act, env_floats, a_stride, l_Rloc, l_w2;
};
constexpr Layout make_layout(int nb, int maxlev, bool alias_w = false) {
  const int nn = nb + 1, nv = 6 + 3 * (nb - 1);
  Layout y{};
  int o = 0;
  auto take = [&](int n) { int r = o; o += (n + 3) & ~3; return r; };
  y.l_q = take(nv + 1); y.l_v = take(nv); y.l_a = take(nv); y.l_tau = take(nv);
  y.l_Fb = take(6 * nb);
  y.l_act = alias_w ? o : take(nv - 6);
  y.l_delta = take(nv);
  y.l_Pb = take(6 * nb);
  y.l_V = y.l_Pb;
  y.l_diag = take(nv);
  y.l_S = take(6 * nv);
  y.l_Ab = take(6 * nb);
  y.l_Iown = take(10 * nb);
  y.l_An = take(8 * nn);
  if (alias_w) {
    y.a_stride = 24;
    y.l_Aown = take(24 * nb);
    y.ia_stride = 0;
    const int gb = (6 * nb + 3) & ~3, t6 = (6 * nn + 3) & ~3;
    y.l_IA = take(48 * maxlev);
    y.l_Gb = y.l_IA;
    y.l_Rloc = y.l_Aown; y.l_tmp = y.l_Aown;
    y.l_w2 = y.l_Aown + 12 * nb;
    y.l_Ubuf = 24 * maxlev <= 8 * nn ? y.l_An : take(24 * maxlev);
    y.l_Wst = y.l_Aown;
    y.l_R = o - 12 * nb; y.l_r = y.l_R + 9 * nb;
    (void)gb; (void)t6;
    y.env_floats = o;
    return y;
  }
  y.a_stride = 21;
  y.l_Aown = take(21 * nb);
  y.ia_stride = 0;
  const int gb = (6 * nb + 3) & ~3;
  const int ia_need = 48 * maxlev > gb + 6 * nn ? 48 * maxlev : gb + 6 * nn;
  y.l_IA = take(ia_need);
  y.l_Gb = y.l_IA; y.l_tmp = y.l_IA + gb;
  y.l_Ubuf = 24 * maxlev <= 8 * nn ? y.l_An : take(24 * maxlev);
  y.l_Wst = take(24 * nn);
  y.l_R = y.l_Wst; y.l_r = y.l_Wst + 9 * nb;
  y.l_Rloc = y.l_IA; y.l_w2 = y.l_Wst + 12 * nb;
  y.env_floats = o;
  return y;
}
constexpr bool alias_layout_fits(int nb, int maxlev, int nslot) {
  const int nn = nb + 1;
  const Layout y = make_layout(nb, maxlev, true);
  return ((6 * nb + 3) & ~3) <= 48 * maxlev && y.l_w2 + ((6 * nn + 3) & ~3) <= y.l_R && 13 * nslot <= y.l_R - y.l_An;
}

constexpr int kMaxSelf = SS_MAX_SELF_CONTACTS;
constexpr int kSelfRec = 24;
constexpr int kSelfCand = 64;
constexpr int kCandRec = 8;
constexpr int kGeomC = 16;
constexpr int kDenseMaxRows = 64;
struct HdrSC {
  int npair;
  int l_H, l_g, l_list, l_Wst2, hloc, o_sctab, l_gc, l_tab, nmax, l_cand, l_zb;
  int env_floats;
};
constexpr int kDenseTile = 16;
constexpr int dense_tile_rows(int nblock) { return (3 * nblock + 1 + kDenseTile - 1) / kDenseTile; }
constexpr int dense_floats(int np) {
  const int t = (np - 1) / kDenseTile;
  return kDenseTile * kDenseTile * (t * (t + 1) / 2) + kDenseTile * (t + 1) * (np - kDenseTile * t);
}
constexpr int kDenseExtra = 256;
constexpr HdrSC make_layout_sc(int nb, int base_floats, int l_An) {
  HdrSC y{};
  int o = base_floats;
  auto take = [&](int n) { int r = o; o += (n + 3) & ~3; return r; };
  y.nmax = nb + 1 < kDenseMaxRows ? nb + 1 : kDenseMaxRows;
  y.l_H = l_An;
  take(kDenseExtra);
  y.hloc = o - y.l_H;
  y.l_g = take(kDenseTile * dense_tile_rows(y.nmax)); y.l_list = take(64);
  const int w2 = 24 * (nb + 1) > kCandRec * kSelfCand ? 24 * (nb + 1) : kCandRec * kSelfCand;
  y.l_Wst2 = take(w2); y.l_cand = y.l_Wst2;
  y.l_gc = take(3 * nb); y.l_zb = take(3 * nb); y.l_tab = take(3 * nb);
  y.env_floats = o;
  return y;
}
constexpr int ss_pool_floats(const HdrSC &y) { return dense_floats(3 * y.nmax + 1) > y.hloc ? 4 + ((dense_floats(3 * y.nmax + 1) + 3) & ~3) : 0; }

struct HdrC {
  int nlev;
  int o_lev;
  int root;
  int pel_level;
  unsigned long long nkpack[2];
  unsigned long long cpack;
  unsigned long long chain;
  unsigned long long neg;
};

#if defined(__HIPCC__)
#define SS_HD __host__ __device__ inline __attribute__((always_inline))
#else
#define SS_HD inline __attribute__((always_inline))
#endif
SS_HD int hdr_o_arm(const Hdr &h) { return (int)(h.arm_lean & 0xffffffffull); }
SS_HD bool hdr_lean(const Hdr &h) { return (h.arm_lean >> 32) != 0ull; }
struct HdrRuntime {
  typedef const Hdr &type;
  static constexpr bool fixed = false;
  static SS_HD bool lean(const Hdr &h) { return hdr_lean(h); }
  static constexpr bool maybe_lean = true;
  static SS_HD type view(const Hdr &h) { return h; }
  typedef const HdrC &tree_type;
  static SS_HD tree_type tree(const HdrC &c) { return c; }
};
template <int NLEV, int ROOT, int PEL, unsigned long long NK0, unsigned long long CP, unsigned long long CH, unsigned long long NG>
struct TreeFixed {
  static constexpr int nlev = NLEV, root = ROOT, pel_level = PEL;
  static constexpr unsigned long long nkpack[2] = {NK0, 0ull};
  static constexpr unsigned long long cpack = CP, chain = CH, neg = NG;
  int o_lev;
};
template <int NB, int MAXLEV, bool ALIAS = false>
struct HdrFixed {
  static constexpr Layout LY = make_layout(NB, MAXLEV, ALIAS);
  static constexpr int nb = NB, nn = NB + 1, nv = 6 + 3 * (NB - 1), nq = 7 + 3 * (NB - 1), maxlev = MAXLEV;
  static constexpr int l_q = LY.l_q, l_v = LY.l_v, l_a = LY.l_a, l_tau = LY.l_tau, l_Fb = LY.l_Fb, l_Pb = LY.l_Pb, l_delta = LY.l_delta,
                       l_diag = LY.l_diag, l_S = LY.l_S, l_Ab = LY.l_Ab, l_An = LY.l_An, l_Aown = LY.l_Aown, l_IA = LY.l_IA,
                       l_Ubuf = LY.l_Ubuf, l_Wst = LY.l_Wst, l_R = LY.l_R, l_r = LY.l_r, l_Gb = LY.l_Gb, l_tmp = LY.l_tmp, l_V = LY.l_V,
                       l_Iown = LY.l_Iown, ia_stride = LY.ia_stride, l_act = LY.l_act, env_floats = LY.env_floats,
                       a_stride = LY.a_stride, l_Rloc = LY.l_Rloc, l_w2 = LY.l_w2;
  const int &nu, &ncand, &nlev, &nbox, &nslot;
  const int &o_dofc, &o_boff, &o_chainnode, &o_ndepth, &o_bparent, &o_sumsmall, &o_sumbig, &o_sumcover, &n_sumsmall, &n_sumbig,
      &shared_words;
  const real &dt, &grav, &margin, &mu;
  const real (&solimp)[5];
  const real &K, &B;
  const real (&qpos0_root)[3];
  SS_HD explicit HdrFixed(const Hdr &h)
      : nu(h.nu), ncand(h.ncand), nlev(h.nlev), nbox(h.nbox), nslot(h.nslot), o_dofc(h.o_dofc),
        o_boff(h.o_boff), o_chainnode(h.o_chainnode), o_ndepth(h.o_ndepth), o_bparent(h.o_bparent),
        o_sumsmall(h.o_sumsmall), o_sumbig(h.o_sumbig), o_sumcover(h.o_sumcover), n_sumsmall(h.n_sumsmall), n_sumbig(h.n_sumbig),
        shared_words(h.shared_words), dt(h.dt), grav(h.grav), margin(h.margin), mu(h.mu), solimp(h.solimp), K(h.K), B(h.B),
        qpos0_root(h.qpos0_root) {}
};
template <int NB, int MAXLEV, int NLEV, int ROOT, int PEL, unsigned long long NK0, unsigned long long CP, unsigned long long CH, unsigned long long NG, bool ALIAS = false, bool LEAN = ALIAS>
struct HdrFixedT {
  typedef const HdrFixed<NB, MAXLEV, ALIAS> type;
  static constexpr bool fixed = true;
  static SS_HD constexpr bool lean(const Hdr &) { return LEAN; }
  static constexpr bool maybe_lean = LEAN;
  static SS_HD HdrFixed<NB, MAXLEV, ALIAS> view(const Hdr &h) { return HdrFixed<NB, MAXLEV, ALIAS>(h); }
  typedef const TreeFixed<NLEV, ROOT, PEL, NK0, CP, CH, NG> tree_type;
  static SS_HD TreeFixed<NLEV, ROOT, PEL, NK0, CP, CH, NG> tree(const HdrC &c) { TreeFixed<NLEV, ROOT, PEL, NK0, CP, CH, NG> t; t.o_lev = c.o_lev; return t; }
  static bool matches(const Hdr &h, const HdrC &c) {
    return h.nb == NB && h.maxlev == MAXLEV && h.a_stride == (ALIAS ? 24 : 21) && hdr_lean(h) == LEAN && h.env_floats == HdrFixed<NB, MAXLEV, ALIAS>::env_floats && c.nlev == NLEV && c.root == ROOT && c.pel_level == PEL && c.nkpack[0] == NK0 && c.nkpack[1] == 0ull && c.cpack == CP && c.chain == CH && c.neg == NG;
  }
};


typedef HdrFixedT<24, 5, 6, 10, 2, 0x333431ull, 0x1253ull, 0x1cull, 0x3ull> HdrSmplFixed;
typedef HdrFixedT<52, 12, 7, 11, 3, 0xbbb3233ull, 0x9a89ull, 0x33ull, 0x7ull, true> HdrSmplxFixed;
typedef HdrFixedT<52, 12, 7, 11, 3, 0xbbb3233ull, 0x9a89ull, 0x33ull, 0x7ull, false, true> HdrSmplxFixedSC;

inline int kernel_variant(const Hdr &h) {
  const int dofp = (h.nv + 63) / 64, candp = (h.ncand + 63) / 64, slotp = (h.nslot + 63) / 64, npass = (h.maxlev + 7) / 8;
  if (dofp <= 2 && candp <= 2 && slotp <= 1 && npass <= 1) return 0;
  if (dofp <= 3 && candp <= 3 && slotp <= 2 && npass <= 2) return 1;
  return -1;
}

template <class H> constexpr int shape_stride(const H &h) { return h.nb * kBodyC + ((h.nv + 3) & ~3); }

enum { MODE_STEP = 0, MODE_SUBSTEP = 1, MODE_RESET = 2, MODE_KINEMATICS = 3, MODE_DEBUG_FORWARD = 4 };

struct KArgs {
  Hdr h;
  ss_env_cfg cfg;
  ss_state st;
  const uint32_t *shared_g;
  const real *bodyc;
  const real *candc;
  const int32_t *candb;
  uint64_t illegal_mask;
  int mode, nsub, obs_size;
  const real *actions;
  const real *task_rand;
  const real *fall_actions;
  const uint8_t *mask;
  unsigned long long *prof;
  const int32_t *order;
  int32_t *work_counter;
  real *obs, *reward;
  int fused_reset;
  real *obs2;
  const real *task_rand2;
  uint8_t *terminated, *truncated;
  real *out0, *out1, *out2;
  HdrSC sc;
  const int32_t *pairs;
  const real *geomc;
  real *dbg_self;
  int obs_stride;
  const void *im;
  const float *im_rand;
  int32_t *work_counter_next;
  real *power;
  int32_t *self_trunc;
  HdrC hc;
};

inline int env_slice_floats(const KArgs &k) { return k.cfg.self_collision ? k.sc.env_floats : k.h.env_floats; }
inline size_t launch_lds_bytes(const KArgs &k, int e) {
  return (size_t)((k.h.shared_words + 3) & ~3) * 4 + ((size_t)e * env_slice_floats(k) + (k.cfg.self_collision ? ss_pool_floats(k.sc) : 0)) * sizeof(real);
}

}
```

smplsim_amd/imitation.py:

```python
import ctypes as C

import torch

from . import _cabi
from .batch import SMPLSimVecEnv, _check, _ptr
from ._lib import lib


class SMPLSimImitationVecEnv:
    def __init__(self, num_envs, motion_lib, model=None, device=0, self_obs_v=2, control_freq_inv=15, sim_timestep_inv=450,
                 termination_distance=0.25, reward_k=(100.0, 10.0, 0.1, 0.1), reward_w=(0.5, 0.3, 0.1, 0.1),
                 random_start=True, autoreset=True, seed=0, fused=True, **env_kw):
        self.base = SMPLSimVecEnv(num_envs, model=model, device=device, task="HumanoidEnv", state_init="External",
                                  self_obs_v=self_obs_v, control_freq_inv=control_freq_inv, episode_length=2 ** 30,
                                  autoreset=False, fused_autoreset=False, seed=seed, **env_kw)
        b = self.base
        self.motion_lib = motion_lib
        if motion_lib.skeleton.num_joints != b.nbody:
            raise ValueError("motion library skeleton and simulated model have different body counts")
        if motion_lib.device != b.device:
            raise ValueError("motion library and env must live on the same device")
        self.num_envs, self.device, self.nbody = b.num_envs, b.device, b.nbody
        self.dt = control_freq_inv / float(sim_timestep_inv)
        self.cfg = _cabi.ImitationCfg(*reward_k, *reward_w, termination_distance, self.dt)
        self.random_start, self.autoreset = random_start, autoreset
        N, J, dev = self.num_envs, self.nbody, self.device
        f32 = dict(dtype=torch.float32, device=dev)
        self.motion_ids = torch.zeros(N, dtype=torch.int32, device=dev)
        self.start_times = torch.zeros(N, **f32)
        self.offset = torch.zeros(N, 3, **f32)
        self.xpos = torch.zeros(N, J, 3, **f32); self.xmat = torch.zeros(N, J, 9, **f32)
        self.self_obs_size, self.task_obs_size = b.obs_size, 24 * J
        self.obs_size = self.self_obs_size + self.task_obs_size
        self.obs_buf = torch.zeros(N, self.obs_size, **f32)
        self.task_obs = self.obs_buf[:, self.self_obs_size:]
        self.rew_buf = torch.zeros(N, **f32)
        self.reward_parts = torch.zeros(N, 4, **f32)
        self.terminated = torch.zeros(N, dtype=torch.uint8, device=dev)
        self.truncated = torch.zeros(N, dtype=torch.uint8, device=dev)
        self.reset_buf = torch.zeros(N, dtype=torch.uint8, device=dev)
        self.action_size = self.nu = b.nu
        self.gen = torch.Generator(device=dev)
        self.gen.manual_seed(int(seed) + 1)
        _check(lib().ss_set_body_outputs(b.handle, _ptr(self.xpos), _ptr(self.xmat)))
        self._rand_block, self._rand_i = None, self.RAND_BLOCK
        self.fused = bool(fused) and not (b.self_collision and (b.shape_id is not None or b.nv > 128))
        self.obs_final = torch.zeros(N, self.obs_size, **f32)
        self._bound = None
        self._bind()

    def _bind(self):
        ml = self.motion_lib
        if not self.fused or self._bound == ml.load_count:
            return
        io = _cabi.ImitationIO(C.pointer(ml.data), self.cfg, *[_ptr(t) for t in (self.motion_ids, self.start_times, self.offset,
                               ml.sampling_cdf)], self.dt, int(bool(self.random_start)), _ptr(self.obs_final), _ptr(self.obs_buf),
                               self.obs_size, _ptr(self.rew_buf), _ptr(self.reward_parts), _ptr(self.terminated), _ptr(self.truncated))
        _check(lib().ss_imitation_bind(self.base.handle, C.byref(io)))
        self._bound = ml.load_count

    RAND_BLOCK = 64

    def _draws(self):
        if self._rand_i >= self.RAND_BLOCK:
            self._rand_block = torch.rand(self.RAND_BLOCK, self.num_envs, 2, device=self.device, generator=self.gen)
            self._rand_i = 0
        self._rand_i += 1
        return self._rand_block[self._rand_i - 1]

    @property
    def times(self):
        return self.start_times + self.base.cur_t.to(torch.float32) * self.dt

    @property
    def motion_len(self):
        return self.motion_lib.get_motion_length(self.motion_ids)

    def _imitation(self, mask, rew, parts, term, trunc):
        b = self.base
        task_ptr = C.c_void_p(self.obs_buf.data_ptr() + 4 * self.self_obs_size)
        _check(lib().ss_imitation_step(C.byref(self.motion_lib.data), C.byref(self.cfg), _ptr(self.motion_ids), _ptr(self.start_times),
                                       _ptr(b.cur_t), _ptr(self.offset), _ptr(mask), self.num_envs, _ptr(self.xpos), _ptr(self.xmat),
                                       _ptr(b.body_vel), task_ptr, self.obs_size, _ptr(rew), _ptr(parts), _ptr(term), _ptr(trunc),
                                       b._stream()))

    def reset(self, mask=None, motion_ids=None, start_times=None, rand=None):
        b, ml = self.base, self.motion_lib
        m = None if mask is None else mask.to(self.device).to(torch.uint8).contiguous()
        if motion_ids is None:
            ml.resample(m, self.motion_ids, self.start_times, truncate_time=self.dt, rand=self._draws() if rand is None else rand)
            if start_times is None and not self.random_start:
                self.start_times.zero_() if m is None else self.start_times.masked_fill_(m.bool(), 0.0)
        else:
            ids = torch.as_tensor(motion_ids, device=self.device).to(torch.int32)
            self.motion_ids.copy_(ids if m is None else torch.where(m.bool(), ids, self.motion_ids))
        if start_times is not None:
            t0 = torch.as_tensor(start_times, device=self.device).to(torch.float32)
            self.start_times.copy_(t0 if m is None else torch.where(m.bool(), t0, self.start_times))
        ml.write_state(self.motion_ids, self.start_times, self.offset, m, b.qpos, b.qvel)
        b.reset(mask=m)
        self._imitation(m, None, None, None, None)
        self.obs_buf[:, :self.self_obs_size] = b.obs_buf
        return self.obs_buf, {"critic_state": self.obs_buf}

    def step(self, actions, _events=None):
        b = self.base
        if self.fused:
            actions = actions.to(torch.float32).contiguous()
            assert actions.shape == (self.num_envs, self.nu) and actions.device == self.device
            rand = self._draws() if self.autoreset else None
            self._keep = (actions, rand)
            self._bind()
            if b.lpt_order:
                _check(lib().ss_schedule_longest_first(b.handle, b._stream()))
            if _events:
                _events[0].record()
            _check(lib().ss_imitation_step_fused(b.handle, _ptr(actions), _ptr(rand), b._stream()))
            if _events:
                _events[1].record()
            if b.lpt_order:
                _check(lib().ss_set_order(b.handle, None))
            return self.obs_buf, self.rew_buf, self.terminated.view(torch.bool), self.truncated.view(torch.bool), \
                {"reward_parts": self.reward_parts, "final_observation": self.obs_final, "critic_state": self.obs_buf}
        b.step(actions)
        self._imitation(None, self.rew_buf, self.reward_parts, self.terminated, self.truncated)
        self.obs_buf[:, :self.self_obs_size] = b.obs_buf
        terminated, truncated = self.terminated.bool(), self.truncated.bool()
        info = {"reward_parts": self.reward_parts}
        if self.autoreset:
            self.obs_final.copy_(self.obs_buf)
            info["final_observation"] = self.obs_final
            torch.bitwise_or(self.terminated, self.truncated, out=self.reset_buf)
            self.reset(mask=self.reset_buf)
        info["critic_state"] = self.obs_buf
        return self.obs_buf, self.rew_buf, terminated, truncated, info

    def reference_actions(self):
        t = self.start_times + (self.base.cur_t.to(torch.float32) + 1.0) * self.dt
        out, _ = self.motion_lib._lookup(self.motion_ids, t, None, False, ["dof_pos"])
        return (out["dof_pos"] / torch.pi).clamp_(-1.0, 1.0)

    @torch.no_grad()
    def evaluate(self, policy=None, max_steps=None):
        from . import metrics
        ml, N = self.motion_lib, self.num_envs
        auto, self.autoreset = self.autoreset, False
        ids = torch.arange(N, device=self.device, dtype=torch.int32) % ml.num_current_motions()
        obs, _ = self.reset(motion_ids=ids, start_times=torch.zeros(N, device=self.device))
        steps = int(max_steps or torch.ceil(self.motion_len.max() / self.dt).item())
        alive = torch.ones(N, dtype=torch.bool, device=self.device)
        finished = torch.zeros(N, dtype=torch.bool, device=self.device)
        pred, ref, valid = [], [], []
        for _ in range(steps):
            act = self.reference_actions() if policy is None else policy(obs)
            obs, _, term, trunc, _ = self.step(act)
            alive &= ~term
            valid.append(alive & ~finished)
            pred.append(self.xpos.clone())
            ref.append(ml._lookup(self.motion_ids, self.times, self.offset, False, ["rg_pos"])[0]["rg_pos"])
            finished |= trunc & alive
        self.autoreset = auto
        pred, ref, valid = torch.stack(pred), torch.stack(ref), torch.stack(valid)
        pp, gg = [], []
        for n in range(N):
            k = int(valid[:, n].sum().item())
            if k >= 3:
                pp.append(pred[:k, n]); gg.append(ref[:k, n])
        out = {"success_rate": float(finished.float().mean().item()), "num_clips": N, "frames_scored": int(valid.sum().item())}
        if pp:
            m = metrics.compute_metrics_lite(pp, gg)
            out.update({k: float(v.mean().item()) for k, v in m.items()})
        return out

    def close(self):
        self.base.close()
```

Before: 2.663 million.

## Compute longest-first env schedule inside the step kernel instead of separate launches

Each wave now computes its env's cost key after finishing the env and atomically bins it into a 1024-bucket histogram. The last wave to finish does a prefix scan and writes the next step's hand-out order into a double-buffered schedule. This removes the separate key and order kernel launches before every step; they remain only as a fallback when the in-launch order is stale. It adds global atomics, a fence per env and a serial tail on the last-finishing wave. It also replaces .bool() copies of the termination flags with zero-copy views.

```diff
diff --git a/include/smplsim_hip.h b/include/smplsim_hip.h
--- a/include/smplsim_hip.h
+++ b/include/smplsim_hip.h
@@ -119,6 +119,8 @@
 
 int ss_set_order(ss_batch *b, const int32_t *order);
 int ss_schedule_longest_first(ss_batch *b, void *stream);
+int ss_set_schedule_in_launch(ss_batch *b, int32_t enable);
+int ss_debug_schedule(ss_batch *b, int32_t *keys, int32_t *order, int32_t *ref_keys, int32_t *ref_order, int32_t *counters, void *stream);
 
 int ss_step_autoreset(ss_batch *b, const float *actions, const float *task_rand, const float *reset_task_rand, float *obs,
                       float *obs_next, float *reward, uint8_t *terminated, uint8_t *truncated, void *stream);
diff --git a/smplsim_amd/_cabi.py b/smplsim_amd/_cabi.py
--- a/smplsim_amd/_cabi.py
+++ b/smplsim_amd/_cabi.py
@@ -118,6 +118,8 @@
     lib.ss_model_elimination_tree.argtypes = [vp, vp, vp, vp, vp, vp]
     lib.ss_step_autoreset.argtypes = [vp] * 10
     lib.ss_schedule_longest_first.argtypes = [vp, vp]
+    lib.ss_set_schedule_in_launch.argtypes = [vp, C.c_int32]
+    lib.ss_debug_schedule.argtypes = [vp, vp, vp, vp, vp, C.POINTER(C.c_int32), vp]
     lib.ss_gae.argtypes = [vp, vp, vp, vp, vp, C.c_int32, C.c_int32, C.c_float, C.c_float, vp, vp, vp]
     lib.ss_debug_prof.argtypes = [vp, vp, C.c_int]
     lib.ss_set_order.argtypes = [vp, vp]
@@ -158,7 +160,7 @@
 
 EXPORTS = ["ss_model_create", "ss_model_create_shapes", "ss_model_destroy", "ss_model_dims", "ss_model_elimination_tree", "ss_obs_size", "ss_batch_create",
            "ss_batch_destroy", "ss_reset", "ss_step", "ss_step_autoreset", "ss_substep", "ss_kinematics", "ss_debug_forward", "ss_debug_self_contacts", "ss_debug_self_truncation",
-           "ss_gae", "ss_debug_prof", "ss_set_order", "ss_set_body_outputs", "ss_set_power_output", "ss_set_launch_geometry", "ss_schedule_longest_first", "ss_launch_info", "ss_last_error",
+           "ss_gae", "ss_debug_prof", "ss_set_order", "ss_set_body_outputs", "ss_set_power_output", "ss_set_launch_geometry", "ss_schedule_longest_first", "ss_set_schedule_in_launch", "ss_debug_schedule", "ss_launch_info", "ss_last_error",
            "ss_model_create_from_mjcf", "ss_model_last_error", "ss_batch_last_error", "ss_imitation_bind", "ss_imitation_step_fused", "ss_get_state", "ss_set_state", "ss_set_fall_actions",
            "ss_motion_cook", "ss_motion_state_at", "ss_motion_resample", "ss_imitation_step"]
 
diff --git a/smplsim_amd/batch.py b/smplsim_amd/batch.py
--- a/smplsim_amd/batch.py
+++ b/smplsim_amd/batch.py
@@ -109,7 +109,7 @@
                  power_scale=1.0, tar_speed=(0.0, 5.0), speed_change=(100, 200), tar_height=(0.5, 1.2),
                  height_change=(100, 200), recovery_steps=60, tar_dist_max=1.0, reach_body="R_Hand", newton_iters=0, fused_autoreset=True,
                  autoreset=True, seed=0, lpt_order=True, shape_id=None, self_collision=False, solver_tolerance=0.0,
-                 **model_kw):
+                 lpt_in_launch=True, **model_kw):
         self.device = _shard_device(device if model is None else model.device)
         self.model = model if model is not None else ShardModel(device=device, control_mode=control_mode, **model_kw)
         mc = self.model.mc
@@ -178,6 +178,8 @@
         self.actuator_names = list(mc.actuator_names)
         self._keep = self._keep2 = None
         self.lpt_order = bool(lpt_order) and N > 64
+        if not lpt_in_launch:
+            _check(lib().ss_set_schedule_in_launch(self.handle, 0))
         self.order = torch.arange(N, dtype=torch.int32, device=dev)
 
     @staticmethod
@@ -232,7 +234,7 @@
                 _check(lib().ss_set_order(self.handle, None))
             info["final_observation"] = self.obs_final
             info["critic_state"] = self.obs_buf
-            return self.obs_buf, self.rew_buf, self.terminated.bool(), self.truncated.bool(), info
+            return self.obs_buf, self.rew_buf, self.terminated.view(torch.bool), self.truncated.view(torch.bool), info
         _check(lib().ss_step(self.handle, _ptr(actions), _ptr(tr), _ptr(self.obs_buf), _ptr(self.rew_buf),
                              _ptr(self.terminated), _ptr(self.truncated), self._stream()))
         if _events:
@@ -247,7 +249,7 @@
             _check(lib().ss_reset(self.handle, _ptr(self.reset_buf), _ptr(fa), _ptr(tr2), _ptr(self.obs_buf),
                                   self._stream()))
         info["critic_state"] = self.obs_buf
-        return self.obs_buf, self.rew_buf, self.terminated.bool(), self.truncated.bool(), info
+        return self.obs_buf, self.rew_buf, self.terminated.view(torch.bool), self.truncated.view(torch.bool), info
 
     def substep(self, actions, n):
         actions = actions.to(torch.float32).contiguous()
@@ -291,6 +293,24 @@
         if warm is not None:
             self.qacc_warm.copy_(as_t(warm))
 
+    def schedule_debug(self, reference=False):
+        N, i32 = self.num_envs, dict(dtype=torch.int32, device=self.device)
+        cnt = (C.c_int32 * 2)()
+        _check(lib().ss_debug_schedule(self.handle, None, None, None, None, cnt, self._stream()))
+        out = {"fresh": bool(cnt[0]), "fallbacks": int(cnt[1])}
+        rec = torch.zeros(N, **i32) if out["fresh"] else None
+        order = torch.zeros(N, **i32) if out["fresh"] else None
+        rk = torch.zeros(N, **i32) if reference else None
+        ro = torch.zeros(N, **i32) if reference else None
+        _check(lib().ss_debug_schedule(self.handle, _ptr(rec), _ptr(order), _ptr(rk), _ptr(ro), None, self._stream()))
+        if out["fresh"]:
+            out["keys"] = (rec >> 22) & 1023
+            out["pos"] = rec & ((1 << 22) - 1)
+            out["order"] = order
+        if reference:
+            out["ref_keys"], out["ref_order"] = rk, ro
+        return out
+
     def launch_info(self):
         a, b, c = C.c_int32(), C.c_int32(), C.c_int32()
         _check(lib().ss_launch_info(self.handle, C.byref(a), C.byref(b), C.byref(c)))
diff --git a/smplsim_amd/csrc/smplsim_hip.hip b/smplsim_amd/csrc/smplsim_hip.hip
--- a/smplsim_amd/csrc/smplsim_hip.hip
+++ b/smplsim_amd/csrc/smplsim_hip.hip
@@ -24,17 +24,8 @@
                                                      int32_t *key) {
   const int env = blockIdx.x * 4 + (threadIdx.x >> 6), lane = threadIdx.x & 63;
   if (env >= n) return;
-  float vm = 0.f, am = 0.f;
-  for (int i = lane; i < nv; i += 64) {
-    const float v = fabsf(qvel[(size_t)env * nv + i]), a = fabsf(qacc[(size_t)env * nv + i]);
-    vm = fmaxf(vm, v == v ? v : 1e6f); am = fmaxf(am, a == a ? a : 1e12f);
-  }
-  for (int m = 32; m >= 1; m >>= 1) { vm = fmaxf(vm, __shfl_xor(vm, m, 64)); am = fmaxf(am, __shfl_xor(am, m, 64)); }
-  if (lane == 0) {
-    const int tc = __popc((unsigned)touch[2 * env]) + __popc((unsigned)touch[2 * env + 1]);
-    const float k = (float)iters[env] + 6.f * (float)tc + 8.f * log1pf(fminf(am, 1e12f)) + 8.f * log1pf(fminf(vm, 1e6f));
-    key[env] = (int32_t)fminf(fmaxf(k, 0.f), 1023.f);
-  }
+  const int k = ss_handout_key(qvel, qacc, touch, iters, nv, env, lane);
+  if (lane == 0) key[env] = k;
 }
 
 __global__ void __launch_bounds__(1024) ss_order_kernel(const int32_t *keys, int32_t *order, int n) {
@@ -82,6 +73,7 @@
   static void free_(void *p) { if (p) (void)hipFree(p); }
   static bool upload(void *dst, const void *src, size_t n) { return hipMemcpy(dst, src, n, hipMemcpyHostToDevice) == hipSuccess; }
   static bool set_device(int d) { return hipSetDevice(d) == hipSuccess; }
+  static constexpr bool inlaunch_order = true;
   static bool download(void *dst, const void *src, size_t n) { return hipMemcpy(dst, src, n, hipMemcpyDeviceToHost) == hipSuccess; }
   static bool copy_d2d(void *dst, const void *src, size_t n, void *stream) { return hipMemcpyAsync(dst, src, n, hipMemcpyDeviceToDevice, (hipStream_t)stream) == hipSuccess; }
   static int lds_capacity() { return 160 * 1024; }
diff --git a/smplsim_amd/csrc/ss_api.h b/smplsim_amd/csrc/ss_api.h
--- a/smplsim_amd/csrc/ss_api.h
+++ b/smplsim_amd/csrc/ss_api.h
@@ -8,6 +8,8 @@
 #include "ss_tables.h"
 
 namespace ss {
+template <class BE, class = void> struct be_inlaunch_order { static constexpr bool value = false; };
+template <class BE> struct be_inlaunch_order<BE, decltype((void)BE::inlaunch_order)> { static constexpr bool value = BE::inlaunch_order; };
 inline std::string &last_error() { static thread_local std::string e; return e; }
 inline std::string *&error_slot() { static thread_local std::string *p = nullptr; return p; }
 struct HandleScope {
@@ -38,6 +40,11 @@
   unsigned long long *d_prof = nullptr;
   const int32_t *order = nullptr;
   int32_t *d_sched = nullptr;
+  mutable int sched_parity = 0;
+  mutable bool sched_fresh = false;
+  bool sched_in_launch = true;
+  int sched_fallbacks = 0;
+  int32_t *order_at(int which) const { return d_sched + ss::sched_order_at(st.num_envs, which); }
   float *body_xpos = nullptr, *body_xmat = nullptr;
   static ss::real *R(float *p) { return reinterpret_cast<ss::real *>(p); }
   static const ss::real *R(const float *p) { return reinterpret_cast<const ss::real *>(p); }
@@ -183,6 +190,7 @@
     if (e < 1) { delete b; return fail(SS_ERR_LDS, "model does not fit in LDS"); }
     { const int mw = BE::max_waves(ss::kernel_variant(h), cfg->self_collision); if (e > mw) e = mw; }
     { const char *cap = getenv("SS_ENVS_PER_WG"); if (cap && atoi(cap) > 0 && atoi(cap) < e) e = atoi(cap); }
+    { const char *sw = getenv("SS_SCHED_IN_LAUNCH"); if (sw && atoi(sw) == 0) b->sched_in_launch = false; }
     b->envs_per_wg = e;
     b->lds_bytes = shared_b + (size_t)e * env_b + pool_b;
 #ifdef SS_PROFILE
@@ -209,6 +217,10 @@
     k.obs_stride = b->obs_size;
     k.prof = b->d_prof;
     k.order = b->order;
+    if (ss::be_inlaunch_order<BE>::value && mode == ss::MODE_STEP && b->sched_in_launch && b->d_sched && b->order == b->order_at(b->sched_parity) &&
+        ss::env_slice_floats(k) >= ss::kSchedBuckets && b->st.num_envs <= (1 << ss::kSchedPosBits)) {
+      k.sched = b->d_sched; k.sched_parity = b->sched_parity;
+    }
     if (mode == ss::MODE_STEP || mode == ss::MODE_RESET) { k.out0 = ss_batch::R(b->body_xpos); k.out1 = ss_batch::R(b->body_xmat); }
     if (mode == ss::MODE_STEP) { k.power = ss_batch::R(b->power); k.self_trunc = b->self_trunc; }
     return k;
@@ -219,6 +231,8 @@
     if (err) return fail(SS_ERR_HIP, err);
     b->kernel_regs = BE::kernel_regs();
     b->parity ^= 1;
+    if (k.sched) { b->sched_parity ^= 1; b->sched_fresh = true; }
+    else if (k.mode != ss::MODE_KINEMATICS) b->sched_fresh = false;
     return SS_OK;
   }
   static int reset(ss_batch *b, const uint8_t *mask, const float *fall_actions, const float *task_rand, float *obs, void *stream) {
@@ -286,12 +300,55 @@
     k.im = b->d_im; k.im_rand = rand;
     return run(b, k, stream);
   }
+  static int sched_alloc(ss_batch *b) {
+    if (b->d_sched) return SS_OK;
+    if (!BE::set_device(b->m->device)) return fail(SS_ERR_HIP, "cannot select device");
+    const size_t words = ss::sched_words(b->st.num_envs);
+    int32_t *p = (int32_t *)BE::alloc(words * sizeof(int32_t));
+    if (!p) return fail(SS_ERR_NOMEM, "device allocation failed");
+    std::vector<int32_t> zeros(words, 0);
+    if (!BE::upload(p, zeros.data(), words * sizeof(int32_t))) { BE::free_(p); return fail(SS_ERR_HIP, "device upload failed"); }
+    b->d_sched = p;
+    return SS_OK;
+  }
+  static int schedule_longest_first(ss_batch *b, void *stream) {
+    if (!b) return fail(SS_ERR_INVALID, "null batch");
+    if (int rc = sched_alloc(b)) return rc;
+    int32_t *ord = b->order_at(b->sched_parity);
+    if (!b->sched_fresh || !b->sched_in_launch) {
+      if (!BE::set_device(b->m->device)) return fail(SS_ERR_HIP, "cannot select device");
+      const char *err = BE::order_by_key(b->st, b->m->hm.h.nv, b->d_sched + ss::kSchedHdr, ord, stream);
+      if (err) return fail(SS_ERR_HIP, err);
+      b->sched_fallbacks++;
+    }
+    b->order = ord;
+    return SS_OK;
+  }
+  static int debug_schedule(ss_batch *b, int32_t *keys, int32_t *order, int32_t *ref_keys, int32_t *ref_order, int32_t *counters, void *stream) {
+    if (!b) return fail(SS_ERR_INVALID, "null batch");
+    if ((!ref_keys) != (!ref_order)) return fail(SS_ERR_INVALID, "pass both reference arrays or neither");
+    if (counters) { counters[0] = (b->sched_fresh && b->sched_in_launch) ? 1 : 0; counters[1] = b->sched_fallbacks; }
+    if (!keys && !order && !ref_keys) return SS_OK;
+    if (!BE::set_device(b->m->device)) return fail(SS_ERR_HIP, "cannot select device");
+    const size_t bytes = (size_t)b->st.num_envs * sizeof(int32_t);
+    if (keys || order) {
+      if (!b->d_sched || !b->sched_fresh) return fail(SS_ERR_INVALID, "the last launch of this batch left no hand-out order");
+      if (keys && !BE::copy_d2d(keys, b->d_sched + ss::kSchedHdr, bytes, stream)) return fail(SS_ERR_HIP, "device copy failed");
+      if (order && !BE::copy_d2d(order, b->order_at(b->sched_parity), bytes, stream)) return fail(SS_ERR_HIP, "device copy failed");
+    }
+    if (ref_keys) {
+      const char *err = BE::order_by_key(b->st, b->m->hm.h.nv, ref_keys, ref_order, stream);
+      if (err) return fail(SS_ERR_HIP, err);
+    }
+    return SS_OK;
+  }
   static int state_field(ss_batch *b, int field, void *buf, bool set, void *stream) {
     if (!b || !buf) return fail(SS_ERR_INVALID, "null argument");
     if (sizeof(ss::real) != sizeof(float)) return fail(SS_ERR_INVALID, "not available in the float64 build");
     const ss::Hdr &h = b->m->hm.h;
     const size_t N = (size_t)b->st.num_envs;
     if (!BE::set_device(b->m->device)) return fail(SS_ERR_HIP, "cannot select device");
+    if (set) b->sched_fresh = false;
     auto copy = [&](void *mine, size_t bytes) { return (set ? BE::copy_d2d(mine, buf, bytes, stream) : BE::copy_d2d(buf, mine, bytes, stream)) ? SS_OK : fail(SS_ERR_HIP, "device copy failed"); };
     switch (field) {
       case SS_FIELD_QPOS: {
@@ -374,7 +431,9 @@
   void ss_batch_destroy(ss_batch *b) { if (b) { BE::free_(b->d_kin); BE::free_(b->d_im); BE::free_(b->d_counter); BE::free_(b->d_prof); BE::free_(b->d_sched); delete b; } }          \
   int ss_set_order(ss_batch *b, const int32_t *order) { ss::HandleScope hs_(b ? &b->err : nullptr);                                                              \
     if (!b) return ss_api<BE>::fail(SS_ERR_INVALID, "null batch");                                                  \
-    b->order = order; return SS_OK;                                                                                  \
+    b->order = order;                                                                                                \
+    if (order) b->sched_fresh = false;      \
+    return SS_OK;                                                                                                    \
   }                                                                                                                  \
   int ss_set_launch_geometry(ss_batch *b, int32_t envs_per_wg, int32_t max_workgroups) { ss::HandleScope hs_(b ? &b->err : nullptr);                              \
     if (!b || envs_per_wg < 0 || envs_per_wg > b->envs_per_wg || max_workgroups < 0)                                   \
@@ -397,14 +456,13 @@
     if (!b) return ss_api<BE>::fail(SS_ERR_INVALID, "null batch");                                                  \
     b->dbg_self = records; return SS_OK;                                                                             \
   }                                                                                                                  \
-  int ss_schedule_longest_first(ss_batch *b, void *stream) { ss::HandleScope hs_(b ? &b->err : nullptr);                                                        \
+  int ss_schedule_longest_first(ss_batch *b, void *stream) { ss::HandleScope hs_(b ? &b->err : nullptr); return ss_api<BE>::schedule_longest_first(b, stream); } \
+  int ss_set_schedule_in_launch(ss_batch *b, int32_t enable) { ss::HandleScope hs_(b ? &b->err : nullptr);                                                        \
     if (!b) return ss_api<BE>::fail(SS_ERR_INVALID, "null batch");                                                  \
-    if (!BE::set_device(b->m->device)) return ss_api<BE>::fail(SS_ERR_HIP, "cannot select device");                  \
-    if (!b->d_sched) b->d_sched = (int32_t *)BE::alloc(2 * sizeof(int32_t) * (size_t)b->st.num_envs);                  \
-    if (!b->d_sched) return ss_api<BE>::fail(SS_ERR_NOMEM, "device allocation failed");                              \
-    const char *err = BE::order_by_key(b->st, b->m->hm.h.nv, b->d_sched + b->st.num_envs, b->d_sched, stream);         \
-    if (err) return ss_api<BE>::fail(SS_ERR_HIP, err);                                                               \
-    b->order = b->d_sched; return SS_OK;                                                                             \
+    b->sched_in_launch = enable != 0; return SS_OK;                                                                  \
+  }                                                                                                                  \
+  int ss_debug_schedule(ss_batch *b, int32_t *keys, int32_t *order, int32_t *ref_keys, int32_t *ref_order, int32_t *counters, void *stream) { \
+    ss::HandleScope hs_(b ? &b->err : nullptr); return ss_api<BE>::debug_schedule(b, keys, order, ref_keys, ref_order, counters, stream);     \
   }                                                                                                                  \
   int ss_gae(const float *rew, const float *nd, const float *ndead, const float *val, const float *boot, int32_t T,   \
              int32_t N, float gamma, float tau, float *adv, float *ret, void *stream) {                             \
diff --git a/smplsim_amd/csrc/ss_env_kernel.h b/smplsim_amd/csrc/ss_env_kernel.h
--- a/smplsim_amd/csrc/ss_env_kernel.h
+++ b/smplsim_amd/csrc/ss_env_kernel.h
@@ -25,6 +25,83 @@
 
 namespace {
 
+__device__ __attribute__((noinline)) float ss_handout_key_sum(float am, float vm, int tc, int it) {
+#pragma clang fp contract(off)
+  return (float)it + 6.f * (float)tc + 8.f * log1pf(fminf(am, 1e12f)) + 8.f * log1pf(fminf(vm, 1e6f));
+}
+__device__ __forceinline__ int ss_handout_key(const float *qvel, const float *qacc, const int32_t *touch, const int32_t *iters, int nv, int env, int lane) {
+  float vm = 0.f, am = 0.f;
+  for (int i = lane; i < nv; i += 64) {
+    const float v = fabsf(qvel[(size_t)env * nv + i]), a = fabsf(qacc[(size_t)env * nv + i]);
+    vm = fmaxf(vm, v == v ? v : 1e6f); am = fmaxf(am, a == a ? a : 1e12f);
+  }
+  for (int m = 32; m >= 1; m >>= 1) { vm = fmaxf(vm, __shfl_xor(vm, m, 64)); am = fmaxf(am, __shfl_xor(am, m, 64)); }
+  const int tc = __popc((unsigned)touch[2 * env]) + __popc((unsigned)touch[2 * env + 1]);
+  const float k = ss_handout_key_sum(am, vm, tc, iters[env]);
+  return (int32_t)fminf(fmaxf(k, 0.f), 1023.f);
+}
+
+#ifdef SS_V_NOINLINE_DONE
+__device__ __attribute__((noinline)) void ss_sched_env_done(const WaveGpu &w, const ss::KArgs &k, int nv, int env) {
+#else
+__device__ __forceinline__ void ss_sched_env_done(const WaveGpu &w, const ss::KArgs &k, int nv, int env) {
+#endif
+#ifdef SS_V_WGFENCE
+  __builtin_amdgcn_fence(__ATOMIC_SEQ_CST, "workgroup");
+#else
+  w.mem_fence();
+#endif
+  const int key = ss_handout_key(k.st.qvel, k.st.qacc_warm, k.st.touch, k.st.solver_iters, nv, env, w.ln);
+  if (w.ln == 0) {
+    const int pos = atomicAdd(k.sched + k.sched_parity * ss::kSchedBuckets + (ss::kSchedBuckets - 1 - key), 1);
+    k.sched[ss::kSchedHdr + env] = (int)(((unsigned)key << ss::kSchedPosBits) | (unsigned)pos);
+  }
+}
+__device__ __forceinline__ void ss_sched_finish(const WaveGpu &w, const ss::KArgs &k, int *offs) {
+  typedef int i32x4 __attribute__((ext_vector_type(4)));
+  const int lane = w.ln, p = k.sched_parity, n = k.st.num_envs;
+  const i32x4 *hist = reinterpret_cast<const i32x4 *>(k.sched + p * ss::kSchedBuckets);
+  i32x4 *twin = reinterpret_cast<i32x4 *>(k.sched + (p ^ 1) * ss::kSchedBuckets);
+  i32x4 hv[4];
+#pragma unroll
+  for (int j = 0; j < 4; j++) hv[j] = hist[4 * lane + j];
+  const i32x4 zero = {0, 0, 0, 0};
+#pragma unroll
+  for (int j = 0; j < 4; j++) twin[4 * lane + j] = zero;
+  if (lane == 0) k.sched[2 * ss::kSchedBuckets + (p ^ 1)] = 0;
+  int total = 0;
+#pragma unroll
+  for (int j = 0; j < 4; j++)
+#pragma unroll
+    for (int c = 0; c < 4; c++) { const int h_ = hv[j][c]; hv[j][c] = total; total += h_; }
+  int incl = total;
+  for (int d = 1; d < 64; d <<= 1) { const int t = __shfl_up(incl, d, 64); if (lane >= d) incl += t; }
+  const int base = incl - total;
+#pragma unroll
+  for (int j = 0; j < 4; j++)
+#pragma unroll
+    for (int c = 0; c < 4; c++) offs[16 * lane + 4 * j + c] = base + hv[j][c];
+  w.sync();
+  const i32x4 *rec = reinterpret_cast<const i32x4 *>(k.sched + ss::kSchedHdr);
+  int32_t *order_next = k.sched + ss::sched_order_at(n, p ^ 1);
+  const int quads = (n + 3) >> 2;
+  for (int q0 = 0; q0 < quads; q0 += 8 * 64) {
+    i32x4 r[8];
+#pragma unroll
+    for (int j = 0; j < 8; j++) { const int q = q0 + 64 * j + lane; r[j] = q < quads ? rec[q] : zero; }
+#pragma unroll
+    for (int j = 0; j < 8; j++) {
+      const int q = q0 + 64 * j + lane;
+#pragma unroll
+      for (int c = 0; c < 4; c++) {
+        const unsigned v = (unsigned)r[j][c];
+        const unsigned at = (unsigned)offs[ss::kSchedBuckets - 1 - (int)(v >> ss::kSchedPosBits)] + (v & ((1u << ss::kSchedPosBits) - 1u));
+        if (q < quads && 4 * q + c < n && at < (unsigned)n) order_next[at] = 4 * q + c;
+      }
+    }
+  }
+}
+
 template <int DOFP, int CANDP, int SLOTP, int NPASS, int MAXT, bool BODYOUT, bool SHAPED, class HT = ss::HdrRuntime, bool SELFCOL = false, bool IMIT = false>
 __global__ void __launch_bounds__(MAXT) ss_env_kernel(const ss::KArgs k) {
   extern __shared__ __align__(16) uint32_t lds[];
@@ -46,6 +123,7 @@
   WaveGpu w{(int)(threadIdx.x & 63)};
   const int total_waves = (int)(gridDim.x * (blockDim.x >> 6));
   bool first = true;
+  int finished = 0;
   for (;;) {
     int env = wave * (int)gridDim.x + (int)blockIdx.x;
     if (!first) {
@@ -65,13 +143,24 @@
         w.sync();
         ss::mo::fused_after_reset(&w, f, env);
       }
-      continue;
+    } else {
+      for (int rep = 0; rep < 2; rep++) {
+        const bool again = ss::run_env<WaveGpu, DOFP, CANDP, SLOTP, NPASS, BODYOUT, SHAPED, HT, SELFCOL>(&w, &k, lds, L, env, mode, pool);
+        w.sync();
+        if (!again) break;
+        mode = ss::MODE_RESET;
+      }
     }
-    for (int rep = 0; rep < 2; rep++) {
-      const bool again = ss::run_env<WaveGpu, DOFP, CANDP, SLOTP, NPASS, BODYOUT, SHAPED, HT, SELFCOL>(&w, &k, lds, L, env, mode, pool);
-      w.sync();
-      if (!again) break;
-      mode = ss::MODE_RESET;
+    if (k.sched) ss_sched_env_done(w, k, HT::view(k.h).nv, env);
+    finished++;
+  }
+  if (k.sched && finished) {
+    __threadfence();
+    int done = 0;
+    if (w.ln == 0) done = atomicAdd(k.sched + 2 * ss::kSchedBuckets + k.sched_parity, finished) + finished;
+    if (__builtin_amdgcn_readfirstlane(done) == k.st.num_envs) {
+      __threadfence();
+      ss_sched_finish(w, k, reinterpret_cast<int *>(L));
     }
   }
 }
diff --git a/smplsim_amd/csrc/ss_hdr.h b/smplsim_amd/csrc/ss_hdr.h
--- a/smplsim_amd/csrc/ss_hdr.h
+++ b/smplsim_amd/csrc/ss_hdr.h
@@ -249,7 +249,16 @@
   real *power;
   int32_t *self_trunc;
   HdrC hc;
-};
+  int32_t *sched;
+  int sched_parity;
+};
+
+constexpr int kSchedBuckets = 1024;
+constexpr int kSchedHdr = 2 * kSchedBuckets + 16;
+constexpr int kSchedPosBits = 22;
+constexpr int sched_rec_words(int n) { return (n + 3) & ~3; }
+constexpr size_t sched_words(int n) { return (size_t)kSchedHdr + 3 * (size_t)sched_rec_words(n); }
+constexpr int sched_order_at(int n, int which) { return kSchedHdr + (1 + which) * sched_rec_words(n); }
 
 inline int env_slice_floats(const KArgs &k) { return k.cfg.self_collision ? k.sc.env_floats : k.h.env_floats; }
 inline size_t launch_lds_bytes(const KArgs &k, int e) {
diff --git a/smplsim_amd/imitation.py b/smplsim_amd/imitation.py
--- a/smplsim_amd/imitation.py
+++ b/smplsim_amd/imitation.py
@@ -125,7 +125,7 @@
         b.step(actions)
         self._imitation(None, self.rew_buf, self.reward_parts, self.terminated, self.truncated)
         self.obs_buf[:, :self.self_obs_size] = b.obs_buf
-        terminated, truncated = self.terminated.bool(), self.truncated.bool()
+        terminated, truncated = self.terminated.view(torch.bool), self.truncated.view(torch.bool)
         info = {"reward_parts": self.reward_parts}
         if self.autoreset:
             self.obs_final.copy_(self.obs_buf)
```

Result: slower. 2.621 million (-1.6%).
